# divyanshu-kumar/openh264-wasm

Hardware: AMD Instinct MI355X
Metric: 1080p30 frames/sec encode+decode per GPU (parity vs oracle; OpenH264 parity unpinned) (higher is better)
Workload: dtype u8

## Files before the change

openh264-wasm_amd/csrc/capi_enc.inc:

```
#include "../../include/h264mi.h"

namespace h264mi {
#define MAX_DECODERS 32
struct DecSlot { DecCtx *c; };
}

struct h264mi_instance {
    h264mi::EncCtx *encoder = nullptr;
    uint8_t *encoded_buffer = nullptr;
    int encoded_buffer_size = 0;
    uint8_t *rgba_dev = nullptr;
    size_t rgba_dev_size = 0;
    h264mi::DecSlot *decoder_pool[MAX_DECODERS] = {};
};

namespace h264mi {
static h264mi_instance g_instance;

static int enc_fetch(h264mi_instance *I, EncCtx *c, int s, uint8_t **out, int *out_size) {
    EncState st;
    if (hipMemcpyAsync(&st, c->d_st + s, sizeof(EncState), hipMemcpyDeviceToHost, c->stream) != hipSuccess) return 0;
    if (hipStreamSynchronize(c->stream) != hipSuccess) return 0;
    if (st.err || st.nal_bytes <= 0) return 0;
    if (I->encoded_buffer_size < st.nal_bytes) {
        free(I->encoded_buffer);
        I->encoded_buffer = (uint8_t *)malloc(st.nal_bytes);
        I->encoded_buffer_size = I->encoded_buffer ? st.nal_bytes : 0;
        if (!I->encoded_buffer) return 0;
    }
    const uint8_t *nal = c->h_desc[c->parity ^ 1][s].nal;
    if (hipMemcpy(I->encoded_buffer, nal, st.nal_bytes, hipMemcpyDeviceToHost) != hipSuccess) return 0;
    *out = I->encoded_buffer;
    *out_size = st.nal_bytes;
    return st.nal_bytes;
}
}

using namespace h264mi;

extern "C" {

int h264mi_i_init_encoder(h264mi_instance *I, int width, int height, int bitrate) {
    if (!I) return -1;
    if (I->encoder) { enc_free(I->encoder); I->encoder = nullptr; }
    I->encoder = enc_create(width, height, bitrate, 1, nullptr);
    return I->encoder ? 0 : -1;
}

void h264mi_i_force_key_frame(h264mi_instance *I) {
    if (I && I->encoder) {
        int one = 1;
        (void)hipMemcpyAsync(&I->encoder->d_st[0].force_idr, &one, sizeof(int), hipMemcpyHostToDevice, I->encoder->stream);
        (void)hipStreamSynchronize(I->encoder->stream);
        printf("Key frame forced.\n");
    }
}

void h264mi_i_encode_frame_yuv_i420(h264mi_instance *I, unsigned char *yuv, int width, int height, unsigned char **out_data,
                                    int *out_size) {
    *out_data = nullptr;
    *out_size = 0;
    EncCtx *c = I ? I->encoder : nullptr;
    if (!c || !yuv || width != c->w || height != c->h) return;
    if (hipMemcpyAsync(c->d_src, yuv, c->fbytes, hipMemcpyHostToDevice, c->stream) != hipSuccess) return;
    if (enc_frame(c, c->d_src) != 0) return;
    enc_fetch(I, c, 0, out_data, out_size);
}

void h264mi_i_encode_frame(h264mi_instance *I, unsigned char *rgba, int width, int height, unsigned char **out_data, int *out_size) {
    *out_data = nullptr;
    *out_size = 0;
    EncCtx *c = I ? I->encoder : nullptr;
    if (!c || !rgba || width != c->w || height != c->h) return;
    size_t n = (size_t)width * height * 4;
    if (I->rgba_dev_size < n) {
        (void)hipFree(I->rgba_dev);
        I->rgba_dev = nullptr; I->rgba_dev_size = 0;
        if (hipMalloc(&I->rgba_dev, n) != hipSuccess) return;
        I->rgba_dev_size = n;
    }
    if (hipMemcpyAsync(I->rgba_dev, rgba, n, hipMemcpyHostToDevice, c->stream) != hipSuccess) return;
    if (launch_rgba_to_i420(I->rgba_dev, width, height, 1, c->d_src, c->stream) != 0) return;
    if (enc_frame(c, c->d_src) != 0) return;
    enc_fetch(I, c, 0, out_data, out_size);
}

int init_encoder(int width, int height, int bitrate) { return h264mi_i_init_encoder(&g_instance, width, height, bitrate); }
void force_key_frame(void) { h264mi_i_force_key_frame(&g_instance); }
void encode_frame_yuv_i420(unsigned char *yuv, int width, int height, unsigned char **out_data, int *out_size) {
    h264mi_i_encode_frame_yuv_i420(&g_instance, yuv, width, height, out_data, out_size);
}
void encode_frame(unsigned char *rgba, int width, int height, unsigned char **out_data, int *out_size) {
    h264mi_i_encode_frame(&g_instance, rgba, width, height, out_data, out_size);
}

void free_buffer(void *ptr) {
    if (ptr != nullptr) free(ptr);
}

struct h264mi_encoder { EncCtx *c; };

h264mi_encoder *h264mi_enc_create(int width, int height, int bitrate, int nstreams, void *hip_stream) {
    EncCtx *c = enc_create(width, height, bitrate, nstreams, (hipStream_t)hip_stream);
    if (!c) return nullptr;
    return new h264mi_encoder{c};
}
void h264mi_enc_destroy(h264mi_encoder *e) {
    if (!e) return;
    (void)hipStreamSynchronize(e->c->stream);
    enc_free(e->c);
    delete e;
}
int h264mi_enc_force_idr(h264mi_encoder *e, int stream) {
    if (!e) return -1;
    int one = 1;
    for (int s = 0; s < e->c->S; s++)
        if (stream < 0 || s == stream)
            if (hipMemcpyAsync(&e->c->d_st[s].force_idr, &one, sizeof(int), hipMemcpyHostToDevice, e->c->stream) != hipSuccess) return -1;
    return hipStreamSynchronize(e->c->stream) == hipSuccess ? 0 : -1;
}
int h264mi_enc_set_frame_skip(h264mi_encoder *e, int enable) {
    if (!e) return -1;
    int v = enable != 0;
    for (int s = 0; s < e->c->S; s++)
        if (hipMemcpyAsync(&e->c->d_st[s].rc.skip_en, &v, sizeof(int), hipMemcpyHostToDevice, e->c->stream) != hipSuccess) return -1;
    return hipStreamSynchronize(e->c->stream) == hipSuccess ? 0 : -1;
}
int h264mi_enc_set_gom_exact(h264mi_encoder *e, int enable) {
    if (!e) return -1;
    if (enable && e->c->slices > 1) return -1;
    e->c->gom_exact = enable != 0;
    return 0;
}
int h264mi_enc_set_slices(h264mi_encoder *e, int n) {
    if (!e || !slices_valid(e->c->mbh, n) || (n > 1 && e->c->gom_exact)) return -1;
    e->c->slices = n;
    return 0;
}
int h264mi_enc_slices(h264mi_encoder *e) { return e ? e->c->slices : -1; }
int h264mi_slice_first_row(int mbh, int n, int k) {
    if (mbh < 1 || !slices_valid(mbh, n) || k < 0 || k > n) return -1;
    return slice_first_row(mbh, n, k);
}
int h264mi_enc_set_quality(h264mi_encoder *e, int enable) { return e ? enc_set_quality(e->c, enable != 0) : -1; }
int h264mi_enc_quality_enabled(h264mi_encoder *e) { return e ? (e->c->quality ? 1 : 0) : -1; }
int h264mi_enc_quality(h264mi_encoder *e, int stream, h264mi_quality *out) {
    if (!e || !out || !e->c->quality || stream < 0 || stream >= e->c->S) return -1;
    if (hipMemcpyAsync(out, e->c->d_qual + stream, sizeof(h264mi_quality), hipMemcpyDeviceToHost, e->c->stream) != hipSuccess) return -1;
    return hipStreamSynchronize(e->c->stream) == hipSuccess ? 0 : -1;
}
const h264mi_quality *h264mi_enc_quality_dev(h264mi_encoder *e) { return e && e->c->quality ? e->c->d_qual : nullptr; }
int h264mi_i420_quality_dev(h264mi_quality *d_out, const void *d_a, const void *d_b, int w, int h, int n, void *hip_stream) {
    if (!d_out || !d_a || !d_b || !quality_args_ok(w, h, n)) return -1;
    return launch_quality_i420(d_out, (const uint8_t *)d_a, (const uint8_t *)d_b, w, h, n, (hipStream_t)hip_stream);
}
double h264mi_psnr(uint64_t sse, uint64_t samples) {
    if (sse == 0) return 100.0;
    return 10.0 * log10(65025.0 * (double)samples / (double)sse);
}
int h264mi_enc_inject_error(h264mi_encoder *e, int stream, int code) {
    if (!e || stream < 0 || stream >= e->c->S || code <= 0) return -1;
    if (hipMemcpyAsync(&e->c->d_st[stream].inject_err, &code, sizeof(int), hipMemcpyHostToDevice, e->c->stream) != hipSuccess) return -1;
    return hipStreamSynchronize(e->c->stream) == hipSuccess ? 0 : -1;
}
int h264mi_enc_frames_skipped(h264mi_encoder *e, int stream) {
    if (!e || stream < 0 || stream >= e->c->S) return -1;
    EncState st;
    if (hipMemcpy(&st, e->c->d_st + stream, sizeof(EncState), hipMemcpyDeviceToHost) != hipSuccess) return -1;
    return st.skipped;
}
static int enc_blend_overlays(EncCtx *c) {
    if (c->ov.empty()) return 0;
    return launch_overlay_i420(c->d_src, c->w, c->h, c->ov_sprites, c->ov_w, c->ov_h, c->ov.data(), (int)c->ov.size(), c->stream);
}
int h264mi_enc_encode(h264mi_encoder *e, const void *d_frames) {
    if (!e || !d_frames) return -1;
    EncCtx *c = e->c;
    if (c->ov.empty()) return enc_frame(c, (const uint8_t *)d_frames);
    if (d_frames != (const void *)c->d_src) {
        const uintptr_t a = (uintptr_t)d_frames, b = (uintptr_t)c->d_src, nb = (uintptr_t)c->S * c->fbytes;
        if (a < b + nb && b < a + nb) return -1;
        if (hipMemcpyAsync(c->d_src, d_frames, nb, hipMemcpyDeviceToDevice, c->stream) != hipSuccess) return -1;
    }
    if (enc_blend_overlays(c) != 0) return -1;
    return enc_frame(c, c->d_src);
}
int h264mi_enc_set_overlays(h264mi_encoder *e, const void *d_sprites, int ow, int oh, int nsprites, const h264mi_overlay *ov, int nov) {
    if (!e) return -1;
    EncCtx *c = e->c;
    if (nov == 0) { c->ov.clear(); c->ov_sprites = nullptr; return 0; }
    if (!d_sprites || !overlay_args_ok(c->w, c->h, c->S, ow, oh, nsprites, ov, nov) ||
        overlay_ranges_overlap(c->d_src, c->w, c->h, c->S, d_sprites, ow, oh, nsprites))
        return -1;
    c->ov.assign(ov, ov + nov);
    c->ov_sprites = (const uint8_t *)d_sprites; c->ov_w = ow; c->ov_h = oh;
    return 0;
}
int h264mi_enc_overlays(h264mi_encoder *e) { return e ? (int)e->c->ov.size() : -1; }
int h264mi_rgba_to_i420a_dev(void *d_dst, const void *d_rgba, int w, int h, int n, void *hip_stream) {
    if (!d_dst || !d_rgba || ((uintptr_t)d_rgba & 3) || !rgba_to_i420a_args_ok(w, h, n)) return -1;
    return launch_rgba_to_i420a((const uint8_t *)d_rgba, w, h, n, (uint8_t *)d_dst, (hipStream_t)hip_stream);
}
int h264mi_i420_overlay_dev(void *d_canvas, int cw, int ch, int ncanvas, const void *d_sprites, int ow, int oh, int nsprites,
                            const h264mi_overlay *ov, int nov, void *hip_stream) {
    if (!d_canvas || !d_sprites || !overlay_args_ok(cw, ch, ncanvas, ow, oh, nsprites, ov, nov) ||
        overlay_ranges_overlap(d_canvas, cw, ch, ncanvas, d_sprites, ow, oh, nsprites))
        return -1;
    return launch_overlay_i420((uint8_t *)d_canvas, cw, ch, (const uint8_t *)d_sprites, ow, oh, ov, nov, (hipStream_t)hip_stream);
}
int h264mi_enc_encode_rgba(h264mi_encoder *e, const void *d_rgba_frames) {
    if (!e || !d_rgba_frames || ((uintptr_t)d_rgba_frames & 3)) return -1;
    EncCtx *c = e->c;
    if (launch_rgba_to_i420((const uint8_t *)d_rgba_frames, c->w, c->h, c->S, c->d_src, c->stream) != 0) return -1;
    if (enc_blend_overlays(c) != 0) return -1;
    return enc_frame(c, c->d_src);
}
int h264mi_i420_scale_dev(void *d_dst, int dw, int dh, const void *d_src, int sw, int sh, int n, void *hip_stream) {
    if (!d_dst || !d_src || !scale_args_ok(dw, dh, sw, sh, n) || scale_ranges_overlap(d_dst, dw, dh, d_src, sw, sh, n)) return -1;
    return launch_scale_i420((uint8_t *)d_dst, dw, dh, (const uint8_t *)d_src, sw, sh, n, (hipStream_t)hip_stream);
}
int h264mi_enc_encode_scaled(h264mi_encoder *e, const void *d_frames, int src_w, int src_h) {
    if (!e || !d_frames) return -1;
    EncCtx *c = e->c;
    if (!scale_args_ok(c->w, c->h, src_w, src_h, c->S) || scale_ranges_overlap(c->d_src, c->w, c->h, d_frames, src_w, src_h, c->S)) return -1;
    if (launch_scale_i420(c->d_src, c->w, c->h, (const uint8_t *)d_frames, src_w, src_h, c->S, c->stream) != 0) return -1;
    if (enc_blend_overlays(c) != 0) return -1;
    return enc_frame(c, c->d_src);
}
int h264mi_i420_compose_dev(void *d_canvas, int cw, int ch, int ncanvas, const void *d_src, int src_w, int src_h, int nsrc,
                            const h264mi_cell *cells, int ncells, void *hip_stream) {
    if (!d_canvas || !d_src || !compose_args_ok(cw, ch, ncanvas, src_w, src_h, nsrc, cells, ncells) ||
        compose_ranges_overlap(d_canvas, cw, ch, ncanvas, d_src, src_w, src_h, nsrc))
        return -1;
    return launch_compose_i420((uint8_t *)d_canvas, cw, ch, (const uint8_t *)d_src, src_w, src_h, cells, ncells, (hipStream_t)hip_stream);
}
int h264mi_i420_fill_dev(void *d_frames, int w, int h, int n, int y, int cb, int cr, void *hip_stream) {
    if (!d_frames || !fill_args_ok(w, h, n, y, cb, cr)) return -1;
    return launch_fill_i420((uint8_t *)d_frames, w, h, n, y, cb, cr, (hipStream_t)hip_stream);
}
int h264mi_mosaic_cells(h264mi_cell *out, int cap, int n, int src_w, int src_h, int cw, int ch) {
    return mosaic_cells(out, cap, n, src_w, src_h, cw, ch);
}
int h264mi_enc_encode_composed(h264mi_encoder *e, const void *d_src, int src_w, int src_h, int nsrc, const h264mi_cell *cells, int ncells,
                               int bg_y, int bg_cb, int bg_cr) {
    if (!e || !d_src) return -1;
    EncCtx *c = e->c;
    if (!compose_args_ok(c->w, c->h, c->S, src_w, src_h, nsrc, cells, ncells) ||
        compose_ranges_overlap(c->d_src, c->w, c->h, c->S, d_src, src_w, src_h, nsrc))
        return -1;
    if (bg_y > 255 || bg_cb > 255 || bg_cr > 255 || (bg_y >= 0 && !fill_args_ok(c->w, c->h, c->S, bg_y, bg_cb, bg_cr))) return -1;
    if (bg_y >= 0 && launch_fill_i420(c->d_src, c->w, c->h, c->S, bg_y, bg_cb, bg_cr, c->stream) != 0) return -1;
    if (launch_compose_i420(c->d_src, c->w, c->h, (const uint8_t *)d_src, src_w, src_h, cells, ncells, c->stream) != 0) return -1;
    if (enc_blend_overlays(c) != 0) return -1;
    return enc_frame(c, c->d_src);
}
int h264mi_i420_upscale_dev(void *d_dst, int dw, int dh, const void *d_src, int sw, int sh, int n, int filter, void *hip_stream) {
    if (!d_dst || !d_src || !upscale_args_ok(dw, dh, sw, sh, n, filter) || upscale_ranges_overlap(d_dst, dw, dh, d_src, sw, sh, n)) return -1;
    return launch_upscale_i420((uint8_t *)d_dst, dw, dh, (const uint8_t *)d_src, sw, sh, n, filter, (hipStream_t)hip_stream);
}
int h264mi_i420_compose_any_dev(void *d_canvas, int cw, int ch, int ncanvas, const void *d_src, int src_w, int src_h, int nsrc,
                                const h264mi_cell *cells, int ncells, int filter, void *hip_stream) {
    if (!d_canvas || !d_src || !compose_any_args_ok(cw, ch, ncanvas, src_w, src_h, nsrc, cells, ncells, filter) ||
        compose_ranges_overlap(d_canvas, cw, ch, ncanvas, d_src, src_w, src_h, nsrc))
        return -1;
    return launch_compose_any_i420((uint8_t *)d_canvas, cw, ch, (const uint8_t *)d_src, src_w, src_h, cells, ncells, filter,
                                   (hipStream_t)hip_stream);
}
int h264mi_speaker_cells(h264mi_cell *out, int cap, int n, int speaker, int src_w, int src_h, int cw, int ch) {
    return speaker_cells(out, cap, n, speaker, src_w, src_h, cw, ch);
}
int h264mi_enc_encode_composed_any(h264mi_encoder *e, const void *d_src, int src_w, int src_h, int nsrc, const h264mi_cell *cells, int ncells,
                                   int filter, int bg_y, int bg_cb, int bg_cr) {
    if (!e || !d_src) return -1;
    EncCtx *c = e->c;
    if (!compose_any_args_ok(c->w, c->h, c->S, src_w, src_h, nsrc, cells, ncells, filter) ||
        compose_ranges_overlap(c->d_src, c->w, c->h, c->S, d_src, src_w, src_h, nsrc))
        return -1;
    if (bg_y > 255 || bg_cb > 255 || bg_cr > 255 || (bg_y >= 0 && !fill_args_ok(c->w, c->h, c->S, bg_y, bg_cb, bg_cr))) return -1;
    if (bg_y >= 0 && launch_fill_i420(c->d_src, c->w, c->h, c->S, bg_y, bg_cb, bg_cr, c->stream) != 0) return -1;
    if (launch_compose_any_i420(c->d_src, c->w, c->h, (const uint8_t *)d_src, src_w, src_h, cells, ncells, filter, c->stream) != 0) return -1;
    if (enc_blend_overlays(c) != 0) return -1;
    return enc_frame(c, c->d_src);
}
const void *h264mi_enc_input_buffer(h264mi_encoder *e) { return e ? e->c->d_src : nullptr; }
size_t h264mi_enc_frame_bytes(h264mi_encoder *e) { return e ? e->c->fbytes : 0; }
size_t h264mi_enc_rgba_frame_bytes(h264mi_encoder *e) { return e ? (size_t)e->c->w * e->c->h * 4 : 0; }
int h264mi_enc_sync(h264mi_encoder *e) { return e && hipStreamSynchronize(e->c->stream) == hipSuccess ? 0 : -1; }
int h264mi_enc_nal_bytes(h264mi_encoder *e, int *out) {
    if (!e) return -1;
    std::vector<EncState> st(e->c->S);
    if (hipMemcpyAsync(st.data(), e->c->d_st, sizeof(EncState) * e->c->S, hipMemcpyDeviceToHost, e->c->stream) != hipSuccess) return -1;
    if (hipStreamSynchronize(e->c->stream) != hipSuccess) return -1;
    int err = 0;
    for (int s = 0; s < e->c->S; s++) { out[s] = st[s].nal_bytes; err |= st[s].err; }
    return err ? -2 : 0;
}
const void *h264mi_enc_nal_ptr(h264mi_encoder *e, int stream) {
    if (!e || stream < 0 || stream >= e->c->S) return nullptr;
    return e->c->h_desc[e->c->parity ^ 1][stream].nal;
}
const void *h264mi_enc_recon_ptr(h264mi_encoder *e, int stream) {
    if (!e || stream < 0 || stream >= e->c->S) return nullptr;
    return e->c->h_desc[e->c->parity ^ 1][stream].dbk[0];
}
int h264mi_enc_ref_planes(h264mi_encoder *e, int stream, void *host_out) {
    if (!e || stream < 0 || stream >= e->c->S) return -1;
    const EncDesc &d = e->c->h_desc[0][stream];
    const size_t lsz = (size_t)d.ps * (e->c->ch + 2 * H264MI_LPADY), csz = (size_t)d.psc * (e->c->ch / 2 + 2 * H264MI_CPADY);
    uint8_t *o = (uint8_t *)host_out;
    if (hipStreamSynchronize(e->c->stream) != hipSuccess) return -1;
    for (int k = 0; k < 4; k++)
        if (hipMemcpy(o + k * lsz, d.pl[k] - (size_t)H264MI_LPADY * d.ps - H264MI_LPADX, lsz, hipMemcpyDeviceToHost) != hipSuccess) return -1;
    for (int k = 0; k < 2; k++)
        if (hipMemcpy(o + 4 * lsz + k * csz, d.plc[k] - (size_t)H264MI_CPADY * d.psc - H264MI_CPADX, csz, hipMemcpyDeviceToHost) != hipSuccess) return -1;
    return 0;
}
int h264mi_enc_last_qp(h264mi_encoder *e, int stream) {
    if (!e || stream < 0 || stream >= e->c->S) return -1;
    EncState st;
    if (hipMemcpy(&st, e->c->d_st + stream, sizeof(EncState), hipMemcpyDeviceToHost) != hipSuccess) return -1;
    return st.cur_qp;
}
int h264mi_enc_rc_state(h264mi_encoder *e, int stream, int *out) {
    if (!e || !out || stream < 0 || stream >= e->c->S) return -1;
    EncState st;
    if (hipStreamSynchronize(e->c->stream) != hipSuccess) return -1;
    if (hipMemcpy(&st, e->c->d_st + stream, sizeof(EncState), hipMemcpyDeviceToHost) != hipSuccess) return -1;
    const RcState &r = st.rc;
    const int v[16] = {st.cur_skip, st.cur_qp, r.avg_qp, r.target, r.remaining, (int)r.fullness, r.continual_skip,
                       (int)r.frame_cmplx, r.min_frame_qp, r.max_frame_qp, r.bpf, r.pframe_num, r.idr_num, r.skip_flag,
                       r.remaining_weights, r.frame_coded_in_vgop};
    memcpy(out, v, sizeof(v));
    return 0;
}
int h264mi_enc_gom_state(h264mi_encoder *e, int stream, int *out, int cap) {
    if (!e || stream < 0 || stream >= e->c->S) return -1;
    const int G = e->c->gom_count;
    if (!out || !e->c->gom_exact) return G;
    if (hipStreamSynchronize(e->c->stream) != hipSuccess) return -1;
    std::vector<uint64_t> g(4 * (size_t)G);
    if (hipMemcpy(g.data(), e->c->h_desc[0][stream].gomst, 8 * g.size(), hipMemcpyDeviceToHost) != hipSuccess) return -1;
    for (int i = 0; i < 4 * G && i < cap; i++) out[i] = (int)(uint32_t)g[i];
    return G;
}
int h264mi_rc_qstep_to_qp(int qstep) {
    static const int32_t thr[52] = {H264MI_RC_QP_THR_LIST};
    if (qstep < 64) return 0;
    int q = 0;
    while (q < 52 && qstep >= thr[q]) q++;
    return q;
}
int h264mi_enc_mbinfo(h264mi_encoder *e, int stream, void *host_out) {
    if (!e || stream < 0 || stream >= e->c->S) return -1;
    return hipMemcpy(host_out, e->c->h_desc[0][stream].info, sizeof(MbInfo) * e->c->nmb, hipMemcpyDeviceToHost) == hipSuccess ? 0 : -1;
}
void *h264mi_enc_stream(h264mi_encoder *e) { return e ? (void *)e->c->stream : nullptr; }
const int *h264mi_enc_nal_size_dev(h264mi_encoder *e, int stream) {
    if (!e || stream < 0 || stream >= e->c->S) return nullptr;
    return &e->c->d_st[stream].nal_bytes;
}
int h264mi_enc_copy_nals(h264mi_encoder *e, void *d_dst, int slot_bytes, int *d_sizes) {
    if (!e || !d_dst || slot_bytes <= 0 || (slot_bytes & 3)) return -1;
    EncCtx *c = e->c;
    hipLaunchKernelGGL(enc_copy_nals_kernel, dim3(64, c->S), dim3(256), 0, c->stream,
                       PackNalLaunch{c->S, c->d_desc[c->parity ^ 1], (uint8_t *)d_dst, slot_bytes, (int32_t *)d_sizes});
    return hipGetLastError() == hipSuccess ? 0 : -1;
}
int h264mi_enc_profile(h264mi_encoder *e, uint64_t *out) {
    if (!e || !e->c->d_prof) return -1;
    return hipMemcpy(out, e->c->d_prof, 64 * sizeof(uint64_t), hipMemcpyDeviceToHost) == hipSuccess ? 0 : -1;
}
const uint32_t *h264mi_enc_rows_counter(h264mi_encoder *e) { return e ? e->c->d_ticket + 32 : nullptr; }
int h264mi_enc_timeline(h264mi_encoder *e, uint64_t *out, int n) {
    if (!e || !e->c->d_tl || n < 4 * e->c->S * e->c->mbh) return -1;
    return hipMemcpy(out, e->c->d_tl, 4 * (size_t)e->c->S * e->c->mbh * sizeof(uint64_t), hipMemcpyDeviceToHost) == hipSuccess ? 0 : -1;
}
int h264mi_enc_set_timing(h264mi_encoder *e, int enable) {
    if (!e) return -1;
    if (hipStreamSynchronize(e->c->stream) != hipSuccess) return -1;
    e->c->timing = enable != 0;
    e->c->ev_used = 0;
    return 0;
}
int h264mi_enc_kernel_time(h264mi_encoder *e, double *ms_total, int *launches) {
    if (!e) return -1;
    EncCtx *c = e->c;
    if (hipStreamSynchronize(c->stream) != hipSuccess) return -1;
    double t = 0;
    for (int i = 0; i + 1 < c->ev_used; i += 2) {
        float ms = 0;
        if (hipEventElapsedTime(&ms, c->ev[i], c->ev[i + 1]) != hipSuccess) return -1;
        t += ms;
    }
    *ms_total = t;
    *launches = c->ev_used / 2;
    return 0;
}

}
```

openh264-wasm_amd/csrc/enc_mb.inc:

```
namespace h264mi {

constexpr int ENC_THREADS = 256;
DEV int e_tid() { int t = threadIdx.x; asm volatile("" : "+v"(t)); return t; }
DEV int e_lane() { return e_tid() & 63; }
DEV int e_wave() { return threadIdx.x >> 6; }

constexpr int WIN_RING = 64, WINC_RING = 32;
constexpr int WIN_STRIDE = WIN_RING + 4, WINC_STRIDE = WINC_RING + 4;
DEV void win_put4(uint8_t *d, u32x4 v) { uint32_t *p = (uint32_t *)d; p[0] = v.x; p[1] = v.y; p[2] = v.z; p[3] = v.w; }
DEV void win_put2(uint8_t *d, u32x2 v) { uint32_t *p = (uint32_t *)d; p[0] = v.x; p[1] = v.y; }
constexpr int ENC_CROSS_THR = 1024;
struct EncLds {
    alignas(16) uint8_t win[4][64 * WIN_STRIDE];
    alignas(16) uint8_t winc[2][32 * WINC_STRIDE];
    alignas(16) uint8_t src[256];
    alignas(16) uint8_t srcc[2][64];
    alignas(16) uint8_t pred[256];
    alignas(16) uint8_t predc[2][64];
    alignas(16) uint8_t rec[256];
    alignas(16) uint8_t recc[2][64];
    uint8_t top[24];
    uint8_t topc[2][12];
    uint8_t left[16], leftc[2][8];
    uint8_t n4[16];
    alignas(16) int16_t lvl[24][16];
    alignas(16) int16_t ldc[16];
    alignas(16) int16_t cdc[2][4];
    int dcraw[24];
    int dcval[24];
    alignas(4) uint8_t nnz[24];
    alignas(4) int8_t i4[16];
    uint32_t gp[3][16];
    int cand[32];
    int pj[2][4];
    int refsk[H264MI_ENC_MAX_MBW];
    int abort_flag;
    int gom_qp;
    Xf xft[16];
    alignas(8) I4Tap i4t[9][16];
};

struct EncLaunch {
    int w, h, mbw, mbh, S;
    const EncDesc *desc;
    uint32_t *ticket;
    const uint8_t *src_base;
    size_t src_stride;
    uint64_t *prof;
    int src_vec;
    const DbkDesc *dbk;
    uint64_t *dprof;
    int dlag;
    int xq = 0;
    uint64_t *tl = nullptr;
    int prio = 0;
    int prof_row = -1;
    int gomr = 0;
    int sgrp = 0;
};

constexpr int HAD[4][4] = {{1, 1, 1, 1}, {1, 1, -1, -1}, {1, -1, -1, 1}, {1, -1, 1, -1}};
constexpr uint8_t INVZZ[16] = {0, 1, 5, 6, 2, 4, 7, 12, 3, 8, 11, 13, 9, 10, 14, 15};
constexpr int SUBDX[8] = {0, 0, -1, 1, -1, 1, -1, 1}, SUBDY[8] = {-1, 1, 0, 0, -1, -1, 1, 1};
constexpr uint32_t pack_sub(const int *v) { uint32_t r = 0; for (int k = 0; k < 8; k++) r |= (uint32_t)(v[k] + 1) << (2 * k); return r; }
constexpr uint32_t SUBDX_P = pack_sub(SUBDX), SUBDY_P = pack_sub(SUBDY);
DEV int sub_dx(int k) { return (int)((SUBDX_P >> (2 * k)) & 3) - 1; }
DEV int sub_dy(int k) { return (int)((SUBDY_P >> (2 * k)) & 3) - 1; }
struct QSel { int p1, dx1, dy1, p2, dx2, dy2; };
constexpr uint8_t QSEL_T[16][6] = {
    {0, 0, 0, 0, 0, 0}, {0, 0, 0, 1, 0, 0}, {1, 0, 0, 1, 0, 0}, {1, 0, 0, 0, 1, 0},
    {0, 0, 0, 2, 0, 0}, {1, 0, 0, 2, 0, 0}, {1, 0, 0, 3, 0, 0}, {1, 0, 0, 2, 1, 0},
    {2, 0, 0, 2, 0, 0}, {2, 0, 0, 3, 0, 0}, {3, 0, 0, 3, 0, 0}, {3, 0, 0, 2, 1, 0},
    {2, 0, 0, 0, 0, 1}, {2, 0, 0, 1, 0, 1}, {3, 0, 0, 1, 0, 1}, {2, 1, 0, 1, 0, 1}};
constexpr uint64_t pack_qsel(int half) {
    uint64_t r = 0;
    for (int i = 0; i < 8; i++) {
        const uint8_t *e = QSEL_T[8 * half + i];
        r |= (uint64_t)(e[0] | e[1] << 2 | e[2] << 3 | e[3] << 4 | e[4] << 6 | e[5] << 7) << (8 * i);
    }
    return r;
}
constexpr uint64_t QSEL_LO = pack_qsel(0), QSEL_HI = pack_qsel(1);
DEV QSel qsel(int idx) {
    const uint32_t e = (uint32_t)(((idx < 8 ? QSEL_LO : QSEL_HI) >> (8 * (idx & 7))) & 255);
    return QSel{(int)(e & 3), (int)((e >> 2) & 1), (int)((e >> 3) & 1), (int)((e >> 4) & 3), (int)((e >> 6) & 1), (int)(e >> 7)};
}

DEV int tap6(int a, int b, int c, int d, int e, int f) { return a - 5 * b + 20 * c + 20 * d - 5 * e + f; }

DEV int Wpl(const EncLds &S, int p, int Y0, int gx, int gy) { return S.win[p][(gy - Y0) * WIN_STRIDE + ((gx + 24) & (WIN_RING - 1))]; }
#define AVG(a, b) (((a) + (b) + 1) >> 1)
DEV int Wsample(const EncLds &S, int Y0, int gx, int gy, int fx, int fy) {
    const QSel q = qsel(fy * 4 + fx);
    return AVG(Wpl(S, q.p1, Y0, gx + q.dx1, gy + q.dy1), Wpl(S, q.p2, Y0, gx + q.dx2, gy + q.dy2));
}

DEV int chroma_mc_sample(const EncLds &S, int mbx, int mvx, int mvy, int pl, int x, int y) {
    const int fx = mvx & 7, fy = mvy & 7;
    const int X = mbx * 8 + (mvx >> 3), Y = (mvy >> 3) + 12;
    const uint8_t *W = S.winc[pl];
    const int r0 = (Y + y) * WINC_STRIDE, r1 = r0 + WINC_STRIDE, c0 = (X + x + 12) & (WINC_RING - 1), c1 = (X + x + 13) & (WINC_RING - 1);
    const int A = W[r0 + c0], B = W[r0 + c1], C = W[r1 + c0], E = W[r1 + c1];
    return ((8 - fx) * (8 - fy) * A + fx * (8 - fy) * B + (8 - fx) * fy * C + fx * fy * E + 32) >> 6;
}
DEV void chroma_mc(EncLds &S, int mbx, int mby, int mvx, int mvy) {
    for (int i = e_tid(); i < 128; i += ENC_THREADS) {
        const int pl = i >> 6, p = i & 63;
        S.predc[pl][p] = (uint8_t)chroma_mc_sample(S, mbx, mvx, mvy, pl, p & 7, p >> 3);
    }
}

}
```

openh264-wasm_amd/csrc/enc_mb_kernel.inc:

```
namespace h264mi {

DEV int code_residual_nodc(EncLds &S, const Xf &X, int qp, int intra, int do_luma, bool recon) {
    const int tid = e_tid(), pos = tid & 15, lane = tid & 63;
    const QuantQP q = make_qqp(qp), qc = make_qqp(c_CHROMA_QP[qp]);
    const int fl = qff(q, X.cls, intra), fc = qff(qc, X.cls, intra), fc0 = intra ? qc.fi0 : qc.fp0;
    const int lb = tid >> 4, lx = (lb & 3) * 4 + (pos & 3), ly = (lb >> 2) * 4 + (pos >> 2);
    if (do_luma) {
        const int pv = S.pred[ly * 16 + lx];
        const int t = xf_fwd(S.src[ly * 16 + lx] - pv, X);
        const int mf = X.cls == 0 ? q.mf0 : (X.cls == 1 ? q.mf1 : q.mf2);
        const int lv = quant1(t, mf, fl);
        S.lvl[lb][X.zz] = (int16_t)lv;
        const uint64_t m = __ballot(lv != 0);
        if (pos == 0) S.nnz[lb] = (int)popc((m >> (16 * (lb & 3))) & 0xffffu);
        if (recon) {
            const int v = X.cls == 0 ? q.v0 : (X.cls == 1 ? q.v1 : q.v2);
            const int r = (xf_inv((lv * v) << q.q6, X) + 32) >> 6;
            S.rec[ly * 16 + lx] = (uint8_t)clip1(pv + r);
        }
    }
    if (tid < 128) {
        const int cp = tid >> 6, cb = (tid >> 4) & 3, cx = (cb & 1) * 4 + (pos & 3), cy = (cb >> 1) * 4 + (pos >> 2);
        const int pv = S.predc[cp][cy * 8 + cx];
        const int t = xf_fwd(S.srcc[cp][cy * 8 + cx] - pv, X);
        const int mf = X.cls == 0 ? qc.mf0 : (X.cls == 1 ? qc.mf1 : qc.mf2);
        const int lvc = pos == 0 ? 0 : quant1(t, mf, fc);
        S.lvl[16 + 4 * cp + cb][X.zz] = (int16_t)lvc;
        const uint64_t mc = __ballot(lvc != 0);
        if (pos == 0) S.nnz[16 + 4 * cp + cb] = (int)popc((mc >> (16 * cb)) & 0xffffu);
        const int a = lane_read(t, 0), b = lane_read(t, 16), e = lane_read(t, 32), g = lane_read(t, 48);
        const int c0 = quant_dc(a + b + e + g, qc.mf0, fc0), c1 = quant_dc(a - b + e - g, qc.mf0, fc0);
        const int c2 = quant_dc(a + b - e - g, qc.mf0, fc0), c3 = quant_dc(a - b - e + g, qc.mf0, fc0);
        if (lane == 0) {
            S.cdc[cp][0] = (int16_t)c0; S.cdc[cp][1] = (int16_t)c1; S.cdc[cp][2] = (int16_t)c2; S.cdc[cp][3] = (int16_t)c3;
        }
        if (recon) {
            const int f = cb == 0 ? c0 + c1 + c2 + c3 : cb == 1 ? c0 - c1 + c2 - c3 : cb == 2 ? c0 + c1 - c2 - c3 : c0 - c1 - c2 + c3;
            const int v = X.cls == 0 ? qc.v0 : (X.cls == 1 ? qc.v1 : qc.v2);
            const int w = pos == 0 ? ((f * qc.v0) << qc.q6) >> 1 : (lvc * v) << qc.q6;
            const int r = (xf_inv(w, X) + 32) >> 6;
            S.recc[cp][cy * 8 + cx] = (uint8_t)clip1(pv + r);
        }
    }
    lds_barrier();
    const int probe = lane < 24 ? S.nnz[lane] : (lane < 32 ? S.cdc[(lane - 24) >> 2][(lane - 24) & 3] : 0);
    const uint32_t nzb = (uint32_t)__ballot(probe != 0);
    const int lum = ((nzb & 0x0033u) ? 1 : 0) | ((nzb & 0x00ccu) ? 2 : 0) | ((nzb & 0x3300u) ? 4 : 0) | ((nzb & 0xcc00u) ? 8 : 0);
    const int cbpc = (nzb & 0x00ff0000u) ? 2 : ((nzb & 0xff000000u) ? 1 : 0);
    return uni(lum | (cbpc << 4));
}
DEV int code_residual(EncLds &S, const Xf &X, int qp, int i16, int intra, int do_luma, bool recon = true) {
    const int tid = e_tid(), pos = tid & 15, lane = tid & 63;
    const QuantQP q = make_qqp(qp), qc = make_qqp(c_CHROMA_QP[qp]);
    const int fl = qff(q, X.cls, intra), fc = qff(qc, X.cls, intra), fc0 = intra ? qc.fi0 : qc.fp0;
    const int lb = tid >> 4, lx = (lb & 3) * 4 + (pos & 3), ly = (lb >> 2) * 4 + (pos >> 2);
    int lv = 0;
    if (do_luma) {
        const int d = S.src[ly * 16 + lx] - S.pred[ly * 16 + lx];
        const int t = xf_fwd(d, X);
        if (i16 && pos == 0) S.dcraw[lb] = t;
        const int mf = X.cls == 0 ? q.mf0 : (X.cls == 1 ? q.mf1 : q.mf2);
        lv = (i16 && pos == 0) ? 0 : quant1(t, mf, fl);
        S.lvl[lb][X.zz] = (int16_t)lv;
        const uint64_t m = __ballot(lv != 0);
        if (pos == 0) S.nnz[lb] = (int)popc((m >> (16 * (lb & 3))) & 0xffffu);
    }
    const bool isc = tid < 128;
    const int cp = (tid >> 6) & 1, cb = (tid >> 4) & 3, cx = (cb & 1) * 4 + (pos & 3), cy = (cb >> 1) * 4 + (pos >> 2);
    int lvc = 0;
    if (isc) {
        const int d = S.srcc[cp][cy * 8 + cx] - S.predc[cp][cy * 8 + cx];
        const int t = xf_fwd(d, X);
        if (pos == 0) S.dcraw[16 + 4 * cp + cb] = t;
        const int mf = X.cls == 0 ? qc.mf0 : (X.cls == 1 ? qc.mf1 : qc.mf2);
        lvc = pos == 0 ? 0 : quant1(t, mf, fc);
        S.lvl[16 + 4 * cp + cb][X.zz] = (int16_t)lvc;
    }
    const uint64_t mc = __ballot(lvc != 0);
    if (isc && pos == 0) S.nnz[16 + 4 * cp + cb] = (int)popc((mc >> (16 * cb)) & 0xffffu);
    lds_barrier();
    if (tid < 16 && i16) {
        const int F = (xf_had(S.dcraw[tid], X) + 1) >> 1;
        S.ldc[X.zz] = (int16_t)quant_dc(F, q.mf0, q.fi0);
    }
    if (tid >= 16 && tid < 24) {
        const int pl = (tid - 16) >> 2, k = (tid - 16) & 3;
        const int a = S.dcraw[16 + 4 * pl], b = S.dcraw[17 + 4 * pl], e = S.dcraw[18 + 4 * pl], g = S.dcraw[19 + 4 * pl];
        const int f = k == 0 ? a + b + e + g : k == 1 ? a - b + e - g : k == 2 ? a + b - e - g : a - b - e + g;
        S.cdc[pl][k] = (int16_t)quant_dc(f, qc.mf0, fc0);
    }
    lds_barrier();
    const int probe = lane < 24 ? S.nnz[lane] : (lane < 32 ? S.cdc[(lane - 24) >> 2][(lane - 24) & 3] : 0);
    const uint64_t nzm = __ballot(probe != 0);
    const uint32_t nzb = (uint32_t)nzm;
    int lum = ((nzb & 0x0033u) ? 1 : 0) | ((nzb & 0x00ccu) ? 2 : 0) | ((nzb & 0x3300u) ? 4 : 0) | ((nzb & 0xcc00u) ? 8 : 0);
    if (i16) lum = lum ? 15 : 0;
    const int cbpc = (nzb & 0x00ff0000u) ? 2 : ((nzb & 0xff000000u) ? 1 : 0);
    const int cbp = uni(lum | (cbpc << 4));
    if (!recon) return cbp;
    if (tid < 16 && i16) S.dcval[tid] = luma_dc_scale(xf_had(S.ldc[X.zz], X), q);
    if (tid >= 16 && tid < 24) {
        const int pl = (tid - 16) >> 2, k = (tid - 16) & 3;
        const int a = S.cdc[pl][0], b = S.cdc[pl][1], e = S.cdc[pl][2], g = S.cdc[pl][3];
        const int f = k == 0 ? a + b + e + g : k == 1 ? a - b + e - g : k == 2 ? a + b - e - g : a - b - e + g;
        S.dcval[16 + 4 * pl + k] = ((f * qc.v0) << qc.q6) >> 1;
    }
    lds_barrier();
    if (do_luma) {
        const int v = X.cls == 0 ? q.v0 : (X.cls == 1 ? q.v1 : q.v2);
        int w = (lv * v) << q.q6;
        if (i16 && pos == 0) w = S.dcval[lb];
        const int r = (xf_inv(w, X) + 32) >> 6;
        S.rec[ly * 16 + lx] = (uint8_t)clip1(S.pred[ly * 16 + lx] + r);
    }
    if (isc) {
        const int v = X.cls == 0 ? qc.v0 : (X.cls == 1 ? qc.v1 : qc.v2);
        int w = (lvc * v) << qc.q6;
        if (pos == 0) w = S.dcval[16 + 4 * cp + cb];
        const int r = (xf_inv(w, X) + 32) >> 6;
        S.recc[cp][cy * 8 + cx] = (uint8_t)clip1(S.predc[cp][cy * 8 + cx] + r);
    }
    lds_barrier();
    return cbp;
}

struct I16Ctx { int dc, a, b, c, has_top, has_left; };
template <class LDS> DEV I16Ctx i16_ctx(const LDS &S, int has_top, int has_left) {
    const int l = e_tid() & 15;
    const int st = S.top[1 + l], sl = S.left[l];
    const int hh = l < 8 ? (l + 1) * (S.top[9 + l] - S.top[7 - l]) : 0;
    const int vv = l < 8 ? (l + 1) * (S.left[8 + l] - (l < 7 ? S.left[6 - l] : S.top[0])) : 0;
    const int sumt = lane_read(group16_sum(st), 0), suml = lane_read(group16_sum(sl), 0);
    const int H = lane_read(group16_sum(hh), 0), V = lane_read(group16_sum(vv), 0);
    I16Ctx r;
    if (has_top && has_left) r.dc = (sumt + suml + 16) >> 5;
    else if (has_left) r.dc = (suml + 8) >> 4;
    else if (has_top) r.dc = (sumt + 8) >> 4;
    else r.dc = 128;
    r.a = uni(16 * (S.left[15] + S.top[16])); r.b = (5 * H + 32) >> 6; r.c = (5 * V + 32) >> 6;
    r.has_top = has_top; r.has_left = has_left;
    return r;
}
template <class LDS> DEV int i16_pred(const LDS &S, const I16Ctx &k, int mode, int x, int y) {
    int vh = mode == 0 ? S.top[1 + x] : S.left[y];
    int pln = clip1((k.a + k.b * (x - 7) + k.c * (y - 7) + 16) >> 5);
    return mode <= 1 ? vh : (mode == 2 ? k.dc : pln);
}
DEV bool i16_avail(const I16Ctx &k, int m) {
    return m == 2 || (m == 0 && k.has_top) || (m == 1 && k.has_left) || (m == 3 && k.has_top && k.has_left);
}
DEV void i16_fill_pred(EncLds &S, const I16Ctx &k, int mode) {
    for (int i = e_tid(); i < 256; i += ENC_THREADS) S.pred[i] = (uint8_t)i16_pred(S, k, mode, i & 15, i >> 4);
    lds_barrier();
}

DEV uint32_t md_i16_order(int flags) {
    switch (flags & 7) {
    case 1: case 5: return 0x20012u;
    case 2: case 6: return 0x20002u;
    case 3: return 0x30210u;
    case 7: return 0x43210u;
    default: return 0x10002u;
    }
}
DEV uint32_t md_chroma_order(int flags) {
    switch (flags & 7) {
    case 1: case 5: return 0x20010u;
    case 2: case 6: return 0x20020u;
    case 3: return 0x30012u;
    case 7: return 0x43012u;
    default: return 0x10000u;
    }
}
__constant__ uint64_t c_MD_I4_IDX4[16] = {
    0x7f7f7afa7f117a10ull, 0x7f7f7fff7f117f11ull, 0x7f7f7afa7f7f7afaull, 0x7f7f7fff7f7f7ffbull, 0x7f7f7afa7f117a14ull,
    0x7f7f7fff7f117f15ull, 0x7f7f7afa7f7f7afeull, 0x7f7f7fff7f7f7fffull, 0x7f7f7afa7f917a10ull, 0x7f7f7fff7f917f11ull,
    0x7f7f7afa7fff7afaull, 0x7f7f7fff7fff7ffbull, 0x7f7f7afa7f917a14ull, 0x7f7f7fff7f917f15ull, 0x7f7f7afa7fff7afeull,
    0x7f7f7fff7fff7fffull};
constexpr uint64_t MD_I4_CNT4 = 0x9431643172314231ull;
__constant__ uint32_t c_MD_I4_LIST4[16] = {0x2u, 0x812u, 0x2u, 0x8012u, 0x2u, 0x812u, 0x2u, 0x0u,
                                           0x2u, 0x812u, 0x7302u, 0x738012u, 0x2u, 0x812u, 0x7302u, 0x0u};
DEV int ue_bits(int v) { return 2 * (31 - __clz(v + 1)) + 1; }
DEV int md_first_min(uint32_t ord, const int *cost, int lam, int *best) {
    const int n = (int)(ord >> 16);
    int b = 0x7fffffff, bm = (int)(ord & 15u);
#pragma unroll
    for (int i = 0; i < 4; i++) {
        const int m = (int)((ord >> (4 * i)) & 15u);
        const int cm = m == 0 ? cost[0] : (m == 1 ? cost[1] : (m == 2 ? cost[2] : cost[3]));
        const int c = cm + lam * ue_bits(m);
        if (i < n && c < b) { b = c; bm = m; }
    }
    *best = b;
    return bm;
}
DEV int i4_choose(const int *c, int ai, int *cost) {
    const int cnt = (int)((MD_I4_CNT4 >> (4 * ai)) & 15u);
    int best, m;
    if (cnt == 7 || cnt == 9) {
        const bool hb = c[1] < c[2];
        best = hb ? c[1] : c[2]; m = hb ? 1 : 2;
        if (c[0] < best) { best = c[0]; m = 0; }
        if (c[0] < c[1]) {
            if (cnt == 9) {
                if (c[5] < best) { best = c[5]; m = 5; }
                if (best > c[7]) { best = c[7]; m = 7; }
                if (!(c[0] <= c[7] && c[0] <= c[5])) {
                    if (c[5] < c[7]) { if (c[4] < best) { best = c[4]; m = 4; } }
                    else if (c[3] < best) { best = c[3]; m = 3; }
                }
            } else {
                if (c[4] < best) { best = c[4]; m = 4; }
                if (c[5] < best) { best = c[5]; m = 5; }
            }
        } else {
            if (c[6] < best) { best = c[6]; m = 6; }
            if (best > c[8]) { best = c[8]; m = 8; }
            if (!(c[6] >= c[1] && c[8] >= c[1])) {
                if (c[8] > c[6]) { if (c[4] < best) { best = c[4]; m = 4; } }
                else if (cnt == 9 && c[3] < best) { best = c[3]; m = 3; }
            }
        }
    } else {
        best = 0x7fffffff; m = 2;
        const uint32_t list = c_MD_I4_LIST4[ai];
        for (int i = 0; i < cnt; i++) {
            const int mm = (int)((list >> (4 * i)) & 15u);
            if (c[mm] < best) { best = c[mm]; m = mm; }
        }
    }
    *cost = best;
    return m;
}
DEV void i16_sad_mode(EncLds &S, const I16Ctx &k, int m) {
    const int lane = e_lane(), blk = lane >> 2, row = lane & 3;
    const int y = (blk >> 2) * 4 + row, x0 = (blk & 3) * 4;
    if (!i16_avail(k, m)) return;
    const uint32_t sv = *(const uint32_t *)&S.src[y * 16 + x0];
    int v = 0;
#pragma unroll
    for (int j = 0; j < 4; j++) v += iabs((int)((sv >> (8 * j)) & 255) - i16_pred(S, k, m, x0 + j, y));
    const int sad = wave_sum(v);
    if (lane == 0) S.cand[20 + m] = sad;
}
DEV int i16_first_min(const EncLds &S, int lam, int flags, int *cost) {
    int c[4];
#pragma unroll
    for (int m = 0; m < 4; m++) c[m] = uni(S.cand[20 + m]);
    return md_first_min(md_i16_order(flags), c, lam, cost);
}
DEV int i16_decide_oh(EncLds &S, const I16Ctx &k, int lam, int flags, int *cost) {
    i16_sad_mode(S, k, uni(e_wave()));
    lds_barrier();
    return i16_first_min(S, lam, flags, cost);
}
DEV int vaa_intra_var(const EncLds &S) {
    const int l = e_lane() & 15, bx = l & 3, by = l >> 2;
    int t = 0;
#pragma unroll
    for (int y = 0; y < 4; y++) {
        const uint32_t w = *(const uint32_t *)&S.src[(4 * by + y) * 16 + 4 * bx];
        t += (int)(w & 255) + (int)((w >> 8) & 255) + (int)((w >> 16) & 255) + (int)(w >> 24);
    }
    const int a = t >> 4;
    const uint32_t sum = (uint32_t)lane_read(group16_sum(a), 0), sq = (uint32_t)lane_read(group16_sum(a * a), 0);
    return (int)(sq - ((sum * sum) >> 4));
}

struct CCtx { int a[2], b[2], c[2], has_top, has_left; };
template <class LDS> DEV CCtx chroma_ctx(const LDS &S, int has_top, int has_left) {
    CCtx r;
    for (int pl = 0; pl < 2; pl++) {
        int H = 0, V = 0;
        for (int i = 0; i < 4; i++) {
            H += (i + 1) * (S.topc[pl][1 + 4 + i] - S.topc[pl][1 + 2 - i]);
            V += (i + 1) * (S.leftc[pl][4 + i] - (2 - i >= 0 ? S.leftc[pl][2 - i] : S.topc[pl][0]));
        }
        r.a[pl] = uni(16 * (S.leftc[pl][7] + S.topc[pl][8])); r.b[pl] = uni((34 * H + 32) >> 6); r.c[pl] = uni((34 * V + 32) >> 6);
    }
    r.has_top = has_top; r.has_left = has_left;
    return r;
}
template <class LDS> DEV int chroma_dc_blk(const LDS &S, const CCtx &k, int pl, int bx, int by) {
    int st = 0, sl = 0;
    for (int i = 0; i < 4; i++) { st += S.topc[pl][1 + 4 * bx + i]; sl += S.leftc[pl][4 * by + i]; }
    int t = k.has_top, l = k.has_left;
    if (bx == by) return (t && l) ? (st + sl + 4) >> 3 : l ? (sl + 2) >> 2 : t ? (st + 2) >> 2 : 128;
    if (bx == 1) return t ? (st + 2) >> 2 : l ? (sl + 2) >> 2 : 128;
    return l ? (sl + 2) >> 2 : t ? (st + 2) >> 2 : 128;
}
template <class LDS> DEV int chroma_pred(const LDS &S, const CCtx &k, int mode, int pl, int x, int y, int dcv) {
    int hv = mode == 1 ? S.leftc[pl][y] : S.topc[pl][1 + x];
    const int ka = pl ? k.a[1] : k.a[0], kb = pl ? k.b[1] : k.b[0], kc = pl ? k.c[1] : k.c[0];
    int pln = clip1((ka + kb * (x - 3) + kc * (y - 3) + 16) >> 5);
    return mode == 0 ? dcv : (mode <= 2 ? hv : pln);
}
DEV bool chroma_avail(const CCtx &k, int m) {
    return m == 0 || (m == 1 && k.has_left) || (m == 2 && k.has_top) || (m == 3 && k.has_top && k.has_left);
}
__device__ __noinline__ int chroma_decide_fill(EncLds &S, int a0, int a1, int b0, int b1, int c0, int c1, int has_top, int has_left,
                                               int lam, int flags) {
    CCtx k;
    k.a[0] = uni(a0); k.a[1] = uni(a1); k.b[0] = uni(b0); k.b[1] = uni(b1); k.c[0] = uni(c0); k.c[1] = uni(c1);
    k.has_top = uni(has_top); k.has_left = uni(has_left);
    int lane = e_lane();
    int m = (lane >> 3) & 3, pl = (lane >> 2) & 1, blk = lane & 3, ox = (blk & 1) * 4, oy = (blk >> 1) * 4;
    int dcv = chroma_dc_blk(S, k, pl, blk & 1, blk >> 1);
    int d[16];
#pragma unroll
    for (int y = 0; y < 4; y++)
#pragma unroll
        for (int x = 0; x < 4; x++) d[4 * y + x] = S.srcc[pl][(oy + y) * 8 + ox + x] - chroma_pred(S, k, m, pl, ox + x, oy + y, dcv);
    int s = 0;
#pragma unroll
    for (int i = 0; i < 16; i++) s += iabs(d[i]);
    s = group8_sum(s);
    int c[4];
#pragma unroll
    for (int mm = 0; mm < 4; mm++) c[mm] = lane_read(s, mm * 8);
    int bc;
    int best = uni(md_first_min(md_chroma_order(uni(flags)), c, uni(lam), &bc));
    for (int i = e_tid(); i < 128; i += ENC_THREADS) {
        int p2 = i >> 6, p = i & 63, x = p & 7, y = p >> 3;
        int dv = chroma_dc_blk(S, k, p2, x >> 2, y >> 2);
        S.predc[p2][p] = (uint8_t)chroma_pred(S, k, best, p2, x, y, dv);
    }
    lds_barrier();
    return best;
}
DEV int chroma_decide_fill(EncLds &S, const CCtx &k, int lam, int flags) {
    return uni(chroma_decide_fill(S, k.a[0], k.a[1], k.b[0], k.b[1], k.c[0], k.c[1], k.has_top, k.has_left, lam, flags));
}

struct MvNb { int avail, ref, mx, my; };
DEV MvNb nb_from_payload(const uint32_t *p, int k, bool avail) {
    MvNb r;
    r.avail = avail;
    if (!avail) { r.ref = -1; r.mx = r.my = 0; return r; }
    r.ref = uni((int8_t)((p[8] >> (k < 2 ? 16 : 24)) & 255));
    r.mx = uni((int16_t)(p[12 + k] & 0xffff)); r.my = uni((int16_t)(p[12 + k] >> 16));
    return r;
}
DEV void mv_pred16(MvNb A, MvNb B, MvNb C, int out[2]) {
    if (!B.avail && !C.avail && A.avail) { B = A; C = A; }
    int n = (A.ref == 0) + (B.ref == 0) + (C.ref == 0);
    if (n == 1) {
        out[0] = A.ref == 0 ? A.mx : (B.ref == 0 ? B.mx : C.mx);
        out[1] = A.ref == 0 ? A.my : (B.ref == 0 ? B.my : C.my);
        return;
    }
    out[0] = median3(A.mx, B.mx, C.mx);
    out[1] = median3(A.my, B.my, C.my);
}
DEV bool me_start_cand(int n, int p0, int p1, int amx, int amy, int bmx, int bmy, int cmx, int cmy, bool okA, bool okB, bool okC,
                       int &cx, int &cy) {
    const int mx = n == 2 ? amx : (n == 3 ? bmx : cmx), my = n == 2 ? amy : (n == 3 ? bmy : cmy);
    const bool ok = n == 2 ? okA : (n == 3 ? okB : okC);
    const int vx = n == 0 ? p0 : (n == 1 ? 0 : mx), vy = n == 0 ? p1 : (n == 1 ? 0 : my);
    cx = clip3(-16, 16, (vx + 2) >> 2); cy = clip3(-16, 16, (vy + 2) >> 2);
    return n < 2 || ok;
}
DEV int mvbits(int mx, int my, const int mvp[2]) { return se_len(mx - mvp[0]) + se_len(my - mvp[1]); }

DEV uint32_t win4(const EncLds &S, int p, int wr, int gx) {
    const int sl = (gx + 24) & 63;
    const uint32_t *row = (const uint32_t *)&S.win[p][wr * WIN_STRIDE];
    return __builtin_amdgcn_alignbyte(row[((sl >> 2) + 1) & 15], row[sl >> 2], sl & 3);
}
DEV int sad16_row_group(const EncLds &S, int Y0, int X, int Y, int cx, int cy) {
    const int row = e_tid() & 15;
    const u32x4 sv = *(const u32x4 *)&S.src[row * 16];
    const int sl = (X + cx + 24) & 63, i0 = sl >> 2, sh = sl & 3;
    const uint32_t *rw = (const uint32_t *)&S.win[0][(Y + cy + row - Y0) * WIN_STRIDE];
    const uint32_t w0 = rw[i0], w1 = rw[(i0 + 1) & 15], w2 = rw[(i0 + 2) & 15], w3 = rw[(i0 + 3) & 15], w4 = rw[(i0 + 4) & 15];
    uint32_t acc = __builtin_amdgcn_sad_u8(sv.x, __builtin_amdgcn_alignbyte(w1, w0, sh), 0u);
    acc = __builtin_amdgcn_sad_u8(sv.y, __builtin_amdgcn_alignbyte(w2, w1, sh), acc);
    acc = __builtin_amdgcn_sad_u8(sv.z, __builtin_amdgcn_alignbyte(w3, w2, sh), acc);
    acc = __builtin_amdgcn_sad_u8(sv.w, __builtin_amdgcn_alignbyte(w4, w3, sh), acc);
    return group16_sum((int)acc);
}
template <int N> DEV void satd16_mv_n(const EncLds &S, int Y0, int X, int Y, const int *mvx, const int *mvy, int *out) {
    const int lane = e_tid() & 63, blk = lane >> 2, row = lane & 3;
    const int y = (blk >> 2) * 4 + row, x0 = (blk & 3) * 4;
    const uint32_t sv = *(const uint32_t *)&S.src[y * 16 + x0];
    const int s1 = (row & 1) ? -1 : 1, s2 = (row & 2) ? -1 : 1;
    int acc[N];
#pragma unroll
    for (int n = 0; n < N; n++) {
        const QSel q = qsel((mvy[n] & 3) * 4 + (mvx[n] & 3));
        const int gx = X + x0 + (mvx[n] >> 2), wr = Y + y + (mvy[n] >> 2) - Y0;
        const uint32_t pa = win4(S, q.p1, wr + q.dy1, gx + q.dx1), pb = win4(S, q.p2, wr + q.dy2, gx + q.dx2);
        const uint32_t pv = (pa | pb) - (((pa ^ pb) & 0xFEFEFEFEu) >> 1);
        const int d0 = (int)(sv & 255) - (int)(pv & 255), d1 = (int)((sv >> 8) & 255) - (int)((pv >> 8) & 255);
        const int d2 = (int)((sv >> 16) & 255) - (int)((pv >> 16) & 255), d3 = (int)(sv >> 24) - (int)(pv >> 24);
        const int a0 = d0 + d1, a1 = d0 - d1, a2 = d2 + d3, a3 = d2 - d3;
        int h0 = a0 + a2, h1 = a1 + a3, h2 = a0 - a2, h3 = a1 - a3;
        h0 = dpp<0xB1>(h0) + s1 * h0; h1 = dpp<0xB1>(h1) + s1 * h1; h2 = dpp<0xB1>(h2) + s1 * h2; h3 = dpp<0xB1>(h3) + s1 * h3;
        h0 = dpp<0x4E>(h0) + s2 * h0; h1 = dpp<0x4E>(h1) + s2 * h1; h2 = dpp<0x4E>(h2) + s2 * h2; h3 = dpp<0x4E>(h3) + s2 * h3;
        int v = iabs(h0) + iabs(h1) + iabs(h2) + iabs(h3);
        v += dpp<0xB1>(v);
        v += dpp<0x4E>(v);
        acc[n] = row == 0 ? (v + 1) >> 1 : 0;
    }
#pragma unroll
    for (int n = 0; n < N; n++) acc[n] = group16_sum(acc[n]);
#pragma unroll
    for (int n = 0; n < N; n++) out[n] = lane_read(acc[n], 0) + lane_read(acc[n], 16) + lane_read(acc[n], 32) + lane_read(acc[n], 48);
}
DEV int satd16_mv(const EncLds &S, int Y0, int X, int Y, int mvx, int mvy) {
    int r;
    satd16_mv_n<1>(S, Y0, X, Y, &mvx, &mvy, &r);
    return r;
}
#define PSKIP_MV_MIN (-29)
#define PSKIP_MV_MAX_LOW 12
#define PSKIP_MAX_LEVEL 1
#define PSKIP_LUMA_CTR_MAX 5
#define PSKIP_CHROMA_CTR_MAX 6
#define PSKIP_SINGLE_CTR 0x56Bu
DEV int single_ctr_lane(int lv, int zz) {
    const int m = group16_sum(lv != 0 ? 1 << zz : 0);
    const int lower = m & ((1 << zz) - 1);
    const int run = lower ? zz - 1 - (31 - __builtin_clz((unsigned)lower)) : zz;
    return lv != 0 ? (int)((PSKIP_SINGLE_CTR >> (2 * run)) & 3u) : 0;
}
DEV int zero_sad_bound(const QuantQP &q) {
    const int t0 = 65535 / q.mf0 - q.fp0, t1 = (65535 / q.mf1 - q.fp1) >> 2, t2 = (65535 / q.mf2 - q.fp2) >> 1;
    return min(t0, min(t1, t2));
}
DEV void pskip_luma(EncLds &S, const Xf &X, const QuantQP &q, int Y0, int MX, int MY, int mvx, int mvy, int lb, int &lsad, int &ctr,
                    bool &rej) {
    const int pos = e_lane() & 15, lx = (lb & 3) * 4 + (pos & 3), ly = (lb >> 2) * 4 + (pos >> 2);
    const int pv = Wsample(S, Y0, MX + lx + (mvx >> 2), MY + ly + (mvy >> 2), mvx & 3, mvy & 3);
    S.pred[ly * 16 + lx] = (uint8_t)pv;
    const int dl = S.src[ly * 16 + lx] - pv;
    const int bs = group16_sum(iabs(dl));
    lsad += lane_read(bs, 0) + lane_read(bs, 16) + lane_read(bs, 32) + lane_read(bs, 48);
    if (__ballot(bs > zero_sad_bound(q)) != 0) {
        const int lv = quant1(xf_fwd(dl, X), qmf(q, X.cls), qff(q, X.cls, 0));
        rej = rej || iabs(lv) > PSKIP_MAX_LEVEL;
#ifndef H264MI_DIAG_NO_CTR
        ctr += wave_sum(single_ctr_lane(lv, X.zz));
#endif
    }
}
DEV void pskip_chroma(EncLds &S, const Xf &X, const QuantQP &qc, int mbx, int mvx, int mvy, int cp, int &sad, bool &rej) {
    const int lane = e_lane(), pos = lane & 15, g = lane >> 4, cx = (g & 1) * 4 + (pos & 3), cy = (g >> 1) * 4 + (pos >> 2);
    const int pc = chroma_mc_sample(S, mbx, mvx, mvy, cp, cx, cy);
    S.predc[cp][cy * 8 + cx] = (uint8_t)pc;
    const int dc = S.srcc[cp][cy * 8 + cx] - pc;
    const int bs = group16_sum(iabs(dc));
    const int ps = lane_read(bs, 0) + lane_read(bs, 16) + lane_read(bs, 32) + lane_read(bs, 48);
    sad += ps;
    const int tdc = 65535 / (qc.mf0 >> 1) - 2 * qc.fp0;
    if (__ballot(bs > zero_sad_bound(qc)) != 0 || ps > tdc) {
        const int t = xf_fwd(dc, X);
        const int lvc = quant1(t, qmf(qc, X.cls), qff(qc, X.cls, 0));
        const int a = lane_read(t, 0), b = lane_read(t, 16), e = lane_read(t, 32), f = lane_read(t, 48);
        const bool dcnz = quant_dc(a + b + e + f, qc.mf0, qc.fp0) != 0 || quant_dc(a - b + e - f, qc.mf0, qc.fp0) != 0 ||
                          quant_dc(a + b - e - f, qc.mf0, qc.fp0) != 0 || quant_dc(a - b - e + f, qc.mf0, qc.fp0) != 0;
#ifndef H264MI_DIAG_NO_CTR
        const int cctr = wave_sum(single_ctr_lane(X.zz > 0 ? lvc : 0, X.zz > 0 ? X.zz - 1 : 0));
#else
        const int cctr = 0;
#endif
        rej = rej || iabs(lvc) > PSKIP_MAX_LEVEL || dcnz || cctr > PSKIP_CHROMA_CTR_MAX;
    }
}
DEV void pskip_publish(int *J, int lsad, int csad, int ctr, bool rej) {
    const int lane = e_lane();
    const bool r = __ballot(rej) != 0;
    if (lane == 0) {
        atomicAdd(&J[1], lsad + csad);
        atomicAdd(&J[3], lsad);
        if (ctr) atomicAdd(&J[2], ctr);
        if (r) atomicOr(&J[0], 1);
    }
}
DEV void pskip_judge_4w(EncLds &S, int *J, const Xf &X, int qp, int Y0, int MX, int MY, int mbx, int mvx, int mvy) {
    const int w = e_wave(), g = e_lane() >> 4;
    const QuantQP q = make_qqp(qp), qc = make_qqp(c_CHROMA_QP[qp]);
    int lsad = 0, csad = 0, ctr = 0;
    bool rej = false;
    pskip_luma(S, X, q, Y0, MX, MY, mvx, mvy, 4 * w + g, lsad, ctr, rej);
    if (w < 2) pskip_chroma(S, X, qc, mbx, mvx, mvy, w, csad, rej);
    pskip_publish(J, lsad, csad, ctr, rej);
}
DEV void pskip_judge_3w(EncLds &S, int *J, const Xf &X, int qp, int Y0, int MX, int MY, int mbx, int mvx, int mvy) {
    const int w = e_wave(), g = e_lane() >> 4;
    const QuantQP q = make_qqp(qp), qc = make_qqp(c_CHROMA_QP[qp]);
    int lsad = 0, csad = 0, ctr = 0;
    bool rej = false;
    pskip_luma(S, X, q, Y0, MX, MY, mvx, mvy, 4 * (w - 1) + g, lsad, ctr, rej);
    if (w == 1) pskip_luma(S, X, q, Y0, MX, MY, mvx, mvy, 12 + g, lsad, ctr, rej);
    else pskip_chroma(S, X, qc, mbx, mvx, mvy, w - 2, csad, rej);
    pskip_publish(J, lsad, csad, ctr, rej);
}
DEV int mb_pred_sad(EncLds &S, int *J, bool judged) {
    if (judged) return uni(J[1]);
    const int tid = e_tid();
    int v = iabs((int)S.src[tid] - (int)S.pred[tid]);
    if (tid < 128) v += iabs((int)S.srcc[tid >> 6][tid & 63] - (int)S.predc[tid >> 6][tid & 63]);
    v = wave_sum(v);
    if ((tid & 63) == 0) atomicAdd(&J[1], v);
    lds_barrier();
    return uni(J[1]);
}
DEV void fill_pred_mv(EncLds &S, int Y0, int X, int Y, int mvx, int mvy) {
    const int i = e_tid();
    S.pred[i] = (uint8_t)Wsample(S, Y0, X + (i & 15) + (mvx >> 2), Y + (i >> 4) + (mvy >> 2), mvx & 3, mvy & 3);
}

#define CAND(k) uni(S.cand[k])
DEV bool p_need1(int lane, bool has_next) {
    const int k = lane & 15;
    return (lane < 16 || (lane < 32 && has_next)) && (k == 8 || k >= 12);
}
#ifndef H264MI_ENC_REC_WAVE
#define H264MI_ENC_REC_WAVE 0
#endif
#ifndef H264MI_ENC_LATE_COMMIT
#define H264MI_ENC_LATE_COMMIT 0
#endif
#ifndef H264MI_ENC_ONEBAR
#define H264MI_ENC_ONEBAR 1
#endif
#ifndef H264MI_ENC_XF_LDS
#define H264MI_ENC_XF_LDS 1
#endif
#ifndef H264MI_ENC_ST2PF
#define H264MI_ENC_ST2PF 0
#endif
#ifndef H264MI_ENC_PH1
#define H264MI_ENC_PH1 1
#endif
#ifndef H264MI_ENC_LATE_PF
#define H264MI_ENC_LATE_PF 0
#endif
#ifndef H264MI_ENC_WPE
#define H264MI_ENC_WPE 4
#endif
template <bool LEAN>
__global__ __launch_bounds__(ENC_THREADS)
__attribute__((amdgpu_waves_per_eu(LEAN && H264MI_ENC_WPE > 0 ? H264MI_ENC_WPE : 1, LEAN && H264MI_ENC_WPE > 0 ? H264MI_ENC_WPE : 8)))
void enc_mb_kernel(EncLaunch a) {
    struct DbkCavlcLds { DbkLds d; CavlcTabs T; CavlcWaveLds w[2]; };
    static_assert(sizeof(DbkCavlcLds) <= sizeof(EncLds), "the deblocking workgroup fits the encoder's LDS");
    __shared__ union { EncLds e; DbkCavlcLds k; } SH;
    EncLds &S = SH.e;
    __shared__ int s_ticket;
    const int wv = threadIdx.x >> 6;
#define tid (LEAN ? e_tid() : (int)threadIdx.x)
#define lane (tid & 63)
    const int xq = a.xq, xqi = xq ? (int)(blockIdx.x & 7) : 0, Sq = xq ? a.S >> 3 : a.S;
    if (tid == 0) s_ticket = (int)atomicAdd(a.ticket + (xq ? 8 + xqi : 0), 1u);
    lds_barrier();
    const int t = uni(s_ticket), lagD = a.dlag;
    int tb, tsq;
    if (a.sgrp > 0 && a.sgrp < Sq) {
        const int per = 2 * a.mbh * a.sgrp, g = t / per, tt = t - g * per, gs = min(a.sgrp, Sq - g * a.sgrp);
        tb = tt / gs;
        tsq = g * a.sgrp + (tt - tb * gs);
    } else {
        tb = t / Sq;
        tsq = t - tb * Sq;
    }
    const int ts = xq ? tsq * 8 + xqi : tsq;
    const int tl_slot = xq ? xqi * 2 * Sq * a.mbh + t : t;
    if (a.tl && threadIdx.x == 0) a.tl[2 * tl_slot] = __builtin_amdgcn_s_memrealtime();
    auto tl_end = [&]() {
        if (a.tl && (threadIdx.x & 63) == 0)
            atomicMax((unsigned long long *)&a.tl[2 * tl_slot + 1], (unsigned long long)__builtin_amdgcn_s_memrealtime());
    };
    bool is_dbk;
    int trow;
    if (a.gomr > 0) {
        const int R = a.gomr, k = min(tb / (2 * R), (a.mbh - 1) / R), rows_k = min(R, a.mbh - k * R), ph = tb - 2 * R * k;
        is_dbk = ph >= rows_k;
        trow = k * R + (is_dbk ? ph - rows_k : ph);
    } else if (lagD <= 0 || lagD >= a.mbh) { is_dbk = tb >= a.mbh; trow = is_dbk ? tb - a.mbh : tb; }
    else if (tb < lagD) { is_dbk = false; trow = tb; }
    else {
        const int k = tb - lagD, m = 2 * (a.mbh - lagD);
        if (k < m) { is_dbk = !(k & 1); trow = is_dbk ? (k >> 1) : lagD + (k >> 1); }
        else { is_dbk = true; trow = (a.mbh - lagD) + (k - m); }
    }
    if (is_dbk) {
        const int dby = trow, dsi = ts;
        if (wv == 3 || dby >= a.mbh) return;
        if (uni(cst(a.desc)[dsi].st->cur_skip)) return;
        if (wv == 0) {
            CONSTANT const DbkDesc &DD = cst(a.dbk)[dsi];
            const DbkLaunch dl{a.mbw, a.mbh, a.S, a.dbk, nullptr, a.dprof};
            CONSTANT const EncDesc &DE = cst(a.desc)[dsi];
            const int nsl = uni(DE.st->cur_slices);
            deblock_row(SH.k.d, dl, DD, dby, DbkSrcGranules{gbl((const uint64_t *)DD.src_gran), a.mbw, dby, (uint32_t)uni((int)*DD.epoch),
                                                            gbl((const uint64_t *)DE.rowq), uni(DE.st->cur_qp),
                                                            slice_row_first(a.mbh, nsl, dby), dby > 0 && slice_row_first(a.mbh, nsl, dby - 1)});
        } else {
            CONSTANT const EncDesc &D = cst(a.desc)[dsi];
            cavlc_row(SH.k.T, SH.k.w[wv - 1], D, a.mbw, a.mbh, dby, wv - 1, 2, (uint32_t)uni((int)D.st->epoch), &D.st->err, a.gomr > 0);
        }
        tl_end();
        return;
    }
    const int mby = trow, sidx = ts;
    if (threadIdx.x == 0) __hip_atomic_fetch_add(a.ticket + 32, 1u, __ATOMIC_RELAXED, __HIP_MEMORY_SCOPE_AGENT);
    if (a.prio == 1) __builtin_amdgcn_s_setprio(1);
    else if (a.prio == 2) __builtin_amdgcn_s_setprio(2);
    else if (a.prio == 3) __builtin_amdgcn_s_setprio(3);
    else if (a.prio == 4 && (trow == 0 || trow == a.mbh - 1)) __builtin_amdgcn_s_setprio(3);
    else if (a.prio == 5 && (trow == 0 || trow == a.mbh - 1)) __builtin_amdgcn_s_setprio(2);
    CONSTANT const EncDesc &D = cst(a.desc)[sidx];
    EncState *st = D.st;
    const uint32_t epoch = (uint32_t)uni((int)st->epoch);
    const int mbw = a.mbw, cw = mbw * 16, ch = a.mbh * 16, w = a.w, h = a.h;
    if (uni(st->cur_skip)) {
        for (int pl = 0; pl < 3; pl++) {
            const int pw = pl ? cw / 2 : cw, rows = pl ? 8 : 16, n4 = pw / 4;
            GLOBAL const uint32_t *rs = (GLOBAL const uint32_t *)(gbl(D.ref[pl]) + (size_t)mby * rows * pw);
            GLOBAL uint32_t *rd = (GLOBAL uint32_t *)(gbl(D.dbk[pl]) + (size_t)mby * rows * pw);
            for (int i = tid; i < rows * n4; i += ENC_THREADS) rd[i] = rs[i];
        }
        GLOBAL const int32_t *ks = gbl(D.sksad_ref);
        GLOBAL int32_t *kd = gbl(D.sksad_cur);
        for (int i = tid; i < mbw; i += ENC_THREADS) kd[mby * mbw + i] = ks[mby * mbw + i];
        if (mby == 0 && tid == 0) kd[mbw * a.mbh] = ks[mbw * a.mbh];
        return;
    }
    const int idr = uni(st->cur_idr), slice_qp = uni(st->cur_qp);
    const int sl_row0 = slice_first_row(a.mbh, uni(st->cur_slices), slice_of_row(a.mbh, uni(st->cur_slices), mby));
    int32_t *abort_word = &st->err;
    int qp;
    if (a.gomr > 0 && !idr) {
        if (wv == 0) {
            const int g = gom_row_qp(D, st, mby, mbw, a.gomr, epoch, abort_word);
            if (lane == 0) S.gom_qp = g < 0 ? slice_qp : g;
        }
        lds_barrier();
        qp = uni(S.gom_qp);
    } else {
        qp = idr ? slice_qp : clip3(uni(st->rc.min_frame_qp), uni(st->rc.max_frame_qp), slice_qp + uni(gbl(D.rowqp)[mby]));
    }
    GLOBAL uint64_t *rowq = gbl(D.rowq);
    bool row_carried = false;
    const QuantQP q = make_qqp(qp);
    const int qpc = c_CHROMA_QP[qp];
    const QuantQP qc = make_qqp(qpc);
    const int lam = c_LAMBDA[qp];
#if H264MI_ENC_XF_LDS
    if (tid < 16) S.xft[tid] = xf_consts(tid);
#define XF (S.xft[e_tid() & 15])
#else
    const Xf XF = xf_consts(tid & 15);
#endif
    const int Y0 = mby * 16 - 24, Y = mby * 16;
    GLOBAL const uint8_t *srcY = gbl(a.src_base) + (size_t)sidx * a.src_stride, *srcU = srcY + (size_t)w * h, *srcV = srcU + (size_t)(w / 2) * (h / 2);
    GLOBAL uint64_t *const grow_prev = mby > sl_row0 ? gbl(D.gran) + (size_t)(mby - 1) * mbw * H264MI_GRANULES_PER_MB : nullptr;
#define above (grow_prev != nullptr)
    GLOBAL uint64_t *grow = gbl(D.gran) + (size_t)mby * mbw * H264MI_GRANULES_PER_MB;
    GLOBAL uint64_t *egr = gbl(D.egran);
    GLOBAL uint32_t *info32 = gbl((uint32_t *)D.info);
    GLOBAL MbCoef *coefg = gbl(D.coef);
    if (tid == 0) S.abort_flag = 0;
    int L_ref = -1, L_mvx = 0, L_mvy = 0;
    bool L_skip = false;
    int L_sksad = -1;
    bool i4_dirty = false;
    GLOBAL const int32_t *skref = gbl(D.sksad_ref) + (size_t)mby * mbw;
    const bool ref_p = !idr && uni(gbl(D.sksad_ref)[mbw * a.mbh]) != 0;
    if (ref_p)
        for (int i = tid; i < mbw; i += ENC_THREADS) S.refsk[i] = skref[i];
    if (mby == 0 && tid == 0) gbl(D.sksad_cur)[mbw * a.mbh] = idr ? 0 : 1;
    uint32_t L_i4 = 0;
    __shared__ uint64_t s_prof[40];
#if defined(H264MI_ENC_PROF_BUILD) || defined(H264MI_ENC_PROF_DETAIL)
    const bool prof = a.prof != nullptr && (a.prof_row < 0 || a.prof_row == mby);
#else
    constexpr bool prof = false;
#endif
    uint64_t t_prev = 0;
    if (prof) { if (tid < 40) s_prof[tid] = 0; t_prev = clock64(); }
    auto stamp = [&](int k, uint64_t t0) {
#ifdef H264MI_ENC_PROF_DETAIL
        if (prof && (threadIdx.x & 63) == 0) atomicAdd((unsigned long long *)&s_prof[k], (unsigned long long)(clock64() - t0));
#endif
    };
    auto lap = [&](int k) { if (prof) { uint64_t tt = clock64(); if (tid == 0) s_prof[k] += tt - t_prev; t_prev = tt; } };
#ifdef H264MI_ENC_FINE
    auto lapf = lap;
#else
    auto lapf = [](int) {};
#endif
    lds_barrier();

    const int ps = D.ps, psc = D.psc;
    GLOBAL const uint8_t *plw = gbl(D.pl[tid >> 6]) + (ptrdiff_t)(Y0 + (tid & 63)) * ps;
    GLOBAL const uint8_t *plcw = gbl(D.plc[(tid >> 5) & 1]) + (ptrdiff_t)(mby * 8 - 12 + (tid & 31)) * psc;
    const bool vsrc = a.src_vec != 0;
    u32x4 pfw = {0, 0, 0, 0}, pfa = {0, 0, 0, 0};
    auto issue_prefetch = [&](int nx) {
        if (!idr) {
            pfw = *(GLOBAL const u32x4 *)(plw + 16 * nx + 24);
            if (wv == 0) pfa.xy = *(GLOBAL const u32x2 *)(plcw + 8 * nx + 12);
        }
        if (vsrc && wv == 1) {
            if (lane < 16) pfa = *(GLOBAL const u32x4 *)(srcY + (size_t)min(Y + lane, h - 1) * w + 16 * nx);
            else if (lane < 32) {
                const int pl = (lane - 16) >> 3, r = (lane - 16) & 7;
                pfa.xy = *(GLOBAL const u32x2 *)((pl ? srcV : srcU) + (size_t)min(mby * 8 + r, h / 2 - 1) * (w / 2) + 8 * nx);
            }
        }
    };
    auto commit_prefetch = [&](int nx) {
        if (!idr) {
            win_put4(&S.win[tid >> 6][(tid & 63) * WIN_STRIDE + ((16 * nx + 48) & 63)], pfw);
            if (wv == 0) win_put2(&S.winc[lane >> 5][(lane & 31) * WINC_STRIDE + ((8 * nx + 24) & 31)], pfa.xy);
        }
        if (vsrc && wv == 1) {
            if (lane < 16) *(u32x4 *)&S.src[lane * 16] = pfa;
            else if (lane < 32) *(u32x2 *)&S.srcc[(lane - 16) >> 3][((lane - 16) & 7) * 8] = pfa.xy;
        }
    };
    auto load_src_bytes = [&](int mbx) {
        const int X = mbx * 16, i = tid;
        int x = min(X + (i & 15), w - 1), y = min(Y + (i >> 4), h - 1);
        S.src[i] = srcY[(size_t)y * w + x];
        if (tid < 128) {
            int pl = tid >> 6, p = tid & 63;
            x = min(mbx * 8 + (p & 7), w / 2 - 1); y = min(mby * 8 + (p >> 3), h / 2 - 1);
            S.srcc[pl][p] = (pl ? srcV : srcU)[(size_t)y * (w / 2) + x];
        }
    };
    if (!idr) {
#pragma unroll
        for (int k = 0; k < 4; k++)
            win_put4(&S.win[tid >> 6][(tid & 63) * WIN_STRIDE + 16 * k], *(GLOBAL const u32x4 *)(plw - 24 + 16 * k));
        if (wv == 0) {
#pragma unroll
            for (int k = 0; k < 4; k++)
                win_put2(&S.winc[lane >> 5][(lane & 31) * WINC_STRIDE + 8 * k], *(GLOBAL const u32x2 *)(plcw - 12 + 8 * k));
        }
    }
    load_src_bytes(0);
    if (tid < 16) { S.left[tid] = 0; S.leftc[tid >> 3][tid & 7] = 0; S.i4[tid] = 2; }
    if (tid < 8) S.pj[tid >> 2][tid & 3] = 0;
    static_assert(sizeof(I4Table) == 9 * 16 * 8, "I4Tap is 8 bytes");
    for (int i = tid; i < 9 * 16 * 2; i += ENC_THREADS) ((uint32_t *)S.i4t)[i] = ((const uint32_t *)&c_I4)[i];
    lds_barrier();

    int mbx_cur = 0;
    auto publish_decision = [&](int ty, int mx, int my, int sk) {
        if (wv == 1 && (lane == 8 || (lane >= 12 && lane < 16))) {
            const bool in = ty == MI_I4 || ty == MI_I16;
            const uint32_t v = lane == 8 ? (uint32_t)ty | ((uint32_t)qp << 8) | (in ? 0xffff0000u : 0u)
                                         : (lane == 13 ? (uint32_t)sk : (uint32_t)(uint16_t)mx | ((uint32_t)(uint16_t)my << 16));
            gran_store(grow + (size_t)mbx_cur * 16 + lane, epoch, v);
        }
    };
    uint64_t top_pf = 0;
    uint64_t st2_pf = 0;
    bool st2_stale = true;
    auto st2_need = [&](int nx) { return lane < 8 || lane == 9 || (nx > 0 && (lane == 19 || lane == 21 || lane == 23)); };
    auto st2_load = [&](int nx) -> uint64_t {
        return st2_need(nx) ? __hip_atomic_load(grow_prev + (size_t)(lane < 16 ? nx : nx - 1) * 16 + (lane & 15), __ATOMIC_RELAXED,
                                                __HIP_MEMORY_SCOPE_AGENT)
                            : 0;
    };
    int pend127 = -1;
    for (int mbx = 0; mbx < mbw; mbx++) {
        const int X = mbx * 16;
        mbx_cur = mbx;
        auto commit_here = [&]() {
            if (H264MI_ENC_LATE_COMMIT && mbx > 0) {
                commit_prefetch(mbx);
                stamp(20 + wv, t_prev);
            }
        };
        if (wv != 0 || !above) commit_here();
        if (above) {
            if (wv == 0) {
                bool ok = true;
                if (idr) {
                    uint32_t v;
                    if (mbx == 0) {
                        ok = gran_wait(grow_prev, 16, epoch, &v, abort_word);
                        if (ok && lane < 16) S.gp[0][lane] = v;
                    }
                    if (ok && mbx + 1 < mbw) {
                        ok = gran_wait(grow_prev + (size_t)(mbx + 1) * 16, 16, epoch, &v, abort_word);
                        if (ok && lane < 16) S.gp[(mbx + 1) % 3][lane] = v;
                    }
                } else {
                    const bool need = p_need1(lane, mbx + 1 < mbw);
#if H264MI_ENC_ST2PF
                    if (mbx == 0) st2_pf = st2_load(0);
#endif
                    if (mbx == 0) top_pf = need ? __hip_atomic_load(grow_prev + lane, __ATOMIC_RELAXED, __HIP_MEMORY_SCOPE_AGENT) : 0;
                    ok = gran_poll(grow_prev + (size_t)mbx * 16 + lane, need, epoch, top_pf, abort_word);
                    if (ok && need) S.gp[(mbx + (lane >> 4)) % 3][lane & 15] = (uint32_t)top_pf;
#if H264MI_ENC_ST2PF
                    {
                        const bool need2 = st2_need(mbx), fresh = (uint32_t)(st2_pf >> 32) == epoch;
                        if (ok && need2 && fresh) S.gp[(lane < 16 ? mbx : mbx - 1) % 3][lane & 15] = (uint32_t)st2_pf;
                        st2_stale = __ballot(need2 && !fresh) != 0;
                    }
#endif
                }
                if (!ok && lane == 0) S.abort_flag = 1;
                commit_here();
            }
            lds_barrier();
            if (S.abort_flag) return;
        }
        lap(mbx == 0 ? 0 : 1);
        const int ref_sk = ref_p ? uni(S.refsk[mbx]) : -1;
        if (mbx + 1 < mbw && (idr || !H264MI_ENC_LATE_PF)) issue_prefetch(mbx + 1);
        if (!vsrc && mbx > 0) load_src_bytes(mbx);
        const bool has_top = above, has_left = mbx > 0, has_tr = above && mbx + 1 < mbw, has_tl = has_top && has_left;
        const int nbf = (int)has_left | ((int)has_top << 1) | ((int)has_tl << 2) | ((int)has_tr << 3);
        const uint32_t *PB = S.gp[mbx % 3], *PC = S.gp[(mbx + 1) % 3], *PD = S.gp[(mbx + 2) % 3];
        auto fill_top = [&](bool all_waves, bool tr) {
            const int i = all_waves ? lane : tid;
            const bool luma = i < 21, chroma = i >= 32 && i < 50;
            const int pl = (i - 32) / 9, k = (i - 32) - 9 * pl;
            const int g = luma ? (i == 0 ? 2 * 16 + 3 : (i <= 16 ? (i - 1) >> 2 : 16 + ((i - 17) >> 2)))
                               : (chroma ? (k == 0 ? 2 * 16 + 5 + 2 * pl : 4 + 2 * pl + ((k - 1) >> 2)) : 0);
            const uint32_t w = S.gp[(mbx + (g >> 4)) % 3][g & 15];
            const int sh = luma ? (i == 0 ? 24 : 8 * ((i - 1) & 3)) : (k == 0 ? 24 : 8 * ((k - 1) & 3));
            const bool av = luma ? (i == 0 ? has_tl : (i <= 16 ? has_top : (has_tr && tr))) : (k == 0 ? has_tl : has_top);
            const uint8_t v = av ? (uint8_t)(w >> sh) : (uint8_t)0;
            if (luma) S.top[i] = v;
            if (chroma) S.topc[pl][k] = v;
        };
        auto poll_above = [&](bool tr) -> bool {
            if (!above || (tr && !has_tr)) return true;
            if (wv == 0 && (tr || !H264MI_ENC_ST2PF || st2_stale)) {
#ifndef H264MI_DIAG_NO_G9
                const bool need = tr ? lane < 4 : (lane < 8 || lane == 9 || (mbx > 0 && (lane == 19 || lane == 21 || lane == 23)));
#else
                const bool need = tr ? lane < 4 : (lane < 8 || (mbx > 0 && (lane == 19 || lane == 21 || lane == 23)));
#endif
                const int nb = tr ? mbx + 1 : (lane < 16 ? mbx : mbx - 1);
                GLOBAL uint64_t *g = grow_prev + (size_t)nb * 16 + (lane & 15);
                uint64_t x = need ? __hip_atomic_load(g, __ATOMIC_RELAXED, __HIP_MEMORY_SCOPE_AGENT) : 0;
                const bool ok = gran_poll(g, need, epoch, x, abort_word);
                if (ok && need) S.gp[nb % 3][lane & 15] = (uint32_t)x;
                if (!ok && lane == 0) S.abort_flag = 1;
            }
            lds_barrier();
            return !S.abort_flag;
        };
        if (idr) fill_top(false, true);
        if (idr || i4_dirty) {
            if (tid < 16) S.i4[tid] = 2;
        }
        if (idr || !vsrc || i4_dirty) lds_barrier();
        i4_dirty = false;

        int type = MI_I16, cbp = 0, i16mode = 0, cmode = 0, mvx = 0, mvy = 0, mvdx = 0, mvdy = 0;
        int cur_sk = -1;
        int *J = S.pj[mbx & 1];
        lap(2);
        bool do_intra = idr;
        I16Ctx k16;
        int m16 = 0, c16 = 0x7fffffff;
        if (idr) {
            k16 = i16_ctx(S, has_top, has_left);
            m16 = i16_decide_oh(S, k16, lam, nbf, &c16);
        } else {
#ifdef H264MI_ISA_MARK
            asm volatile(";;MARK_PSTART" ::: "memory");
#endif
            MvNb A, B, C;
            A.avail = has_left;
            if (has_left) { A.ref = L_ref; A.mx = L_mvx; A.my = L_mvy; } else { A.ref = -1; A.mx = A.my = 0; }
            B = nb_from_payload(PB, 0, has_top);
            C = has_tr ? nb_from_payload(PC, 0, true) : nb_from_payload(PD, 3, has_tl);
            int mvp[2], skmv[2] = {0, 0};
            mv_pred16(A, B, C, mvp);
            if (has_left && has_top && !(A.ref == 0 && A.mx == 0 && A.my == 0) && !(B.ref == 0 && B.mx == 0 && B.my == 0)) {
                skmv[0] = mvp[0]; skmv[1] = mvp[1];
            }
            const bool skA = has_left && L_skip, skB = has_top && (uni((int)PB[8]) & 255) == MI_PSKIP;
            const bool skC = has_tr && (uni((int)PC[8]) & 255) == MI_PSKIP, skD = has_tl && (uni((int)PD[8]) & 255) == MI_PSKIP;
            const bool ref_skip = ref_p && ref_sk >= 0;
            const int sx = (skmv[0] >> 2) + 16 * mbx, sy = (skmv[1] >> 2) + 16 * mby;
#ifndef H264MI_DIAG_ALWAYS_TRY
            const bool try_skip = (skA || skB || skC || skD || ref_skip) && sx >= PSKIP_MV_MIN && sx <= ((16 * mbw) | PSKIP_MV_MAX_LOW) &&
                                  sy >= PSKIP_MV_MIN && sy <= ((16 * a.mbh) | PSKIP_MV_MAX_LOW);
#else
            const bool try_skip = true;
#endif
            auto pskip_take = [&]() -> bool {
                const int sA = skA ? L_sksad : 0, sB = skB ? uni((int)PB[13]) : 0;
                const bool skCC = has_tr ? skC : skD;
                const int sC = skCC ? uni((int)(has_tr ? PC[13] : PD[13])) : 0;
                const int f = (int)skA | ((int)skB << 1) | ((int)skCC << 2);
                const int pred = (!has_top && !has_tl && has_left) ? sA : (f == 1 ? sA : (f == 2 ? sB : (f == 4 ? sC : median3(sA, sB, sC))));
                const int tsad = uni(J[1]);
                const bool res_ok = uni(J[0]) == 0 && uni(J[2]) <= PSKIP_LUMA_CTR_MAX;
                return tsad == 0 || tsad < pred || (ref_skip && tsad < ref_sk) || res_ok;
            };
            const bool pred_skip = has_left ? L_skip : skB;
            const bool beside = try_skip && !pred_skip;
            bool skip_taken = false;
            if (H264MI_ENC_LATE_PF == 2 && mbx + 1 < mbw) issue_prefetch(mbx + 1);
#ifdef H264MI_ISA_MARK
            asm volatile(";;MARK_JUDGE" ::: "memory");
#endif
            if (try_skip && pred_skip) {
                pskip_judge_4w(S, J, XF, qp, Y0, X, Y, mbx, skmv[0], skmv[1]);
                lds_barrier();
                skip_taken = pskip_take();
            }
            const bool me_ran = !skip_taken;
            if (!skip_taken) {
                if (!poll_above(false)) return;
#if H264MI_ENC_PH1 == 0
                fill_top(false, false);
                lds_barrier();
                k16 = i16_ctx(S, has_top, has_left);
#elif H264MI_ENC_PH1 == 1
                fill_top(true, false);
                k16 = i16_ctx(S, has_top, has_left);
#endif
#ifdef H264MI_ENC_PROF_DETAIL
                const uint64_t t_ph = prof ? clock64() : 0;
#else
                const uint64_t t_ph = 0;
#endif
                if (wv != 0) {
#if H264MI_ENC_PH1 == 0
                    if (beside) pskip_judge_3w(S, J, XF, qp, Y0, X, Y, mbx, skmv[0], skmv[1]);
                    i16_sad_mode(S, k16, uni(wv - 1));
                    if (wv == (beside ? 3 : 1)) i16_sad_mode(S, k16, 3);
#else
                    if (beside) {
                        pskip_judge_3w(S, J, XF, qp, Y0, X, Y, mbx, skmv[0], skmv[1]);
                        stamp(24 + wv, t_ph);
#if H264MI_ENC_PH1 == 2
                        fill_top(true, false);
                        k16 = i16_ctx(S, has_top, has_left);
#endif
                        if (wv == 1) i16_sad_mode(S, k16, 1);
                        stamp(28 + wv, t_ph);
                        if (wv == 1) i16_sad_mode(S, k16, 0);
                        else if (wv == 3) i16_sad_mode(S, k16, 3);
                        stamp(32 + wv, t_ph);
                    } else {
#if H264MI_ENC_PH1 == 2
                        fill_top(true, false);
                        k16 = i16_ctx(S, has_top, has_left);
#endif
                        i16_sad_mode(S, k16, uni(wv - 1));
                        if (wv == 1) i16_sad_mode(S, k16, 3);
                    }
#endif
                } else {
                    const int grp = (tid >> 4) & 3;
                    int bx, by, bc;
                    {
                        const bool okA = A.avail & (A.ref == 0), okB = B.avail & (B.ref == 0), okC = C.avail & (C.ref == 0);
                        const int amx = A.mx, amy = A.my, bmx = B.mx, bmy = B.my, cmx = C.mx, cmy = C.my, p0 = mvp[0], p1 = mvp[1];
                        auto cand_xy = [&](int n, int &cx, int &cy) -> bool {
                            return me_start_cand(n, p0, p1, amx, amy, bmx, bmy, cmx, cmy, okA, okB, okC, cx, cy);
                        };
                        int cx, cy;
                        bool av = cand_xy(grp, cx, cy);
                        int cost = sad16_row_group(S, Y0, X, Y, cx, cy) + lam * mvbits(4 * cx, 4 * cy, mvp);
                        int k = wave_min(av ? (cost << 3) | grp : 0x7fffffff);
                        if (uni((int)okC)) {
                            av = cand_xy(4, cx, cy) && grp == 0;
                            cost = sad16_row_group(S, Y0, X, Y, cx, cy) + lam * mvbits(4 * cx, 4 * cy, mvp);
                            k = min(k, wave_min(av ? (cost << 3) | 4 : 0x7fffffff));
                        }
                        bc = k >> 3;
                        cand_xy(k & 7, bx, by);
                    }
                    if (beside) stamp(24, t_ph);
                    lapf(12);
                    for (int it = 0; it < 32; it++) {
                        const int cx = bx + (grp == 1 ? -1 : (grp == 2 ? 1 : 0)), cy = by + (grp == 0 ? -1 : (grp == 3 ? 1 : 0));
                        const int sad = sad16_row_group(S, Y0, X, Y, cx, cy);
                        const bool ok = cx >= -16 && cx <= 16 && cy >= -16 && cy <= 16;
                        const int k = wave_min(ok ? ((sad + lam * mvbits(4 * cx, 4 * cy, mvp)) << 2) | grp : 0x7fffffff);
                        if (k == 0x7fffffff || (k >> 2) >= bc) break;
                        bc = k >> 2;
                        bx += (k & 3) == 1 ? -1 : ((k & 3) == 2 ? 1 : 0);
                        by += (k & 3) == 0 ? -1 : ((k & 3) == 3 ? 1 : 0);
                    }
                    if (lane == 0) { S.cand[17] = bx; S.cand[18] = by; S.cand[19] = bc; }
#if H264MI_ENC_PH1 == 2
                    fill_top(true, false);
                    k16 = i16_ctx(S, has_top, has_left);
#endif
#if H264MI_ENC_PH1 != 0
                    if (beside) {
                        stamp(28, t_ph);
                        i16_sad_mode(S, k16, 2);
                        stamp(32, t_ph);
                    }
#endif
                }
#ifndef H264MI_ENC_FINE
                if (prof && lane == 0) atomicAdd((unsigned long long *)&s_prof[11 + wv], (unsigned long long)(clock64() - t_prev));
#endif
                lds_barrier();
                if (beside) skip_taken = pskip_take();
            }
            if (H264MI_ENC_LATE_PF == 1 && mbx + 1 < mbw) issue_prefetch(mbx + 1);
            lap(3);
#ifndef H264MI_DIAG_NO_SKIP_INTRA
            if (skip_taken && !(skA && skB && skC)) {
#else
            if (false) {
#endif
                if (!me_ran) {
                    if (!poll_above(false)) return;
                    fill_top(true, false);
                    k16 = i16_ctx(S, has_top, has_left);
                    i16_sad_mode(S, k16, uni(wv));
                    lds_barrier();
                }
                m16 = i16_first_min(S, lam, nbf, &c16);
                do_intra = c16 < uni(J[3]);
            }
            if (skip_taken && !do_intra) {
                type = MI_PSKIP; mvx = skmv[0]; mvy = skmv[1]; cbp = 0;
                cur_sk = uni(J[1]);
                publish_decision(type, mvx, mvy, cur_sk);
            } else if (!skip_taken) {
                int bx = uni(S.cand[17]), by = uni(S.cand[18]), bcf = uni(S.cand[19]);
                if (uni(S.cand[19]) > ENC_CROSS_THR) {
                    const int bc = uni(S.cand[19]);
                    int kl = 0x7fffffff;
#pragma unroll 1
                    for (int pass = 0; pass < 4; pass++) {
                        const int j = pass * 16 + ((tid >> 4) & 15), hz = j < 32, i = hz ? j : j - 32;
                        const int t = i - 16 + (i - 16 >= (hz ? bx : by) ? 1 : 0);
                        const int cx = hz ? t : bx, cy = hz ? by : t, k = hz ? t + 16 : t + 49;
                        const int sad = sad16_row_group(S, Y0, X, Y, cx, cy);
                        kl = min(kl, ((sad + lam * mvbits(4 * cx, 4 * cy, mvp)) << 7) | k);
                    }
                    const int kmin = wave_min(kl);
                    if (lane == 0) S.cand[24 + wv] = kmin;
                    lds_barrier();
                    const int km = min(min(uni(S.cand[24]), uni(S.cand[25])), min(uni(S.cand[26]), uni(S.cand[27])));
                    if ((km >> 7) < bc) {
                        const int k = km & 127;
                        if (k < 33) bx = k - 16; else by = k - 49;
                        bcf = km >> 7;
                    }
                }
                lap(4);
                m16 = i16_first_min(S, lam, nbf, &c16);
                do_intra = c16 < bcf;
              if (!do_intra) {
                const int wv4 = uni(tid >> 6);
                {
                    int mx[3], my[3], cv[3];
#pragma unroll
                    for (int n = 0; n < 3; n++) {
                        const int k = wv4 + 4 * n - 1;
                        mx[n] = 4 * bx + (k < 0 ? 0 : 2 * sub_dx(k & 7)); my[n] = 4 * by + (k < 0 ? 0 : 2 * sub_dy(k & 7));
                    }
                    if (wv4 == 0) {
                        satd16_mv_n<3>(S, Y0, X, Y, mx, my, cv);
                        if (lane == 0) { S.cand[0] = cv[0]; S.cand[4] = cv[1]; S.cand[8] = cv[2]; }
                    } else {
                        satd16_mv_n<2>(S, Y0, X, Y, mx, my, cv);
                        if (lane == 0) { S.cand[wv4] = cv[0]; S.cand[wv4 + 4] = cv[1]; }
                    }
                }
                lds_barrier();
                lapf(13);
                int bdx, bdy, sc;
                {
                    const int k = lane - 1, ddx = lane == 0 ? 0 : 2 * sub_dx(k & 7), ddy = lane == 0 ? 0 : 2 * sub_dy(k & 7);
                    const int key = lane < 9 ? ((S.cand[lane] + lam * mvbits(4 * bx + ddx, 4 * by + ddy, mvp)) << 4) | lane : 0x7fffffff;
                    const int m = wave_min(key), o = m & 15;
                    sc = m >> 4;
                    bdx = o == 0 ? 0 : 2 * sub_dx(o - 1); bdy = o == 0 ? 0 : 2 * sub_dy(o - 1);
                }
                {
                    int mx[2], my[2], cv[2];
#pragma unroll
                    for (int n = 0; n < 2; n++) { mx[n] = 4 * bx + bdx + sub_dx(wv4 + 4 * n); my[n] = 4 * by + bdy + sub_dy(wv4 + 4 * n); }
                    satd16_mv_n<2>(S, Y0, X, Y, mx, my, cv);
                    if (lane == 0) { S.cand[9 + wv4] = cv[0]; S.cand[13 + wv4] = cv[1]; }
                }
                lds_barrier();
                lapf(14);
                {
                    const int ddx = bdx + sub_dx(lane & 7), ddy = bdy + sub_dy(lane & 7);
                    const int key = lane < 8 ? ((S.cand[9 + lane] + lam * mvbits(4 * bx + ddx, 4 * by + ddy, mvp)) << 4) | (lane + 1)
                                             : (lane == 8 ? sc << 4 : 0x7fffffff);
                    const int m = wave_min(key), o = m & 15;
                    sc = m >> 4;
                    if (o > 0) { bdx += sub_dx(o - 1); bdy += sub_dy(o - 1); }
                }
                lap(5);
                {
                    type = MI_P16x16;
                    mvx = 4 * bx + bdx; mvy = 4 * by + bdy;
                    const bool at_skmv = mvx == skmv[0] && mvy == skmv[1];
                    if (!at_skmv) publish_decision(type, mvx, mvy, -1);
                    mvdx = mvx - mvp[0]; mvdy = mvy - mvp[1];
                    fill_pred_mv(S, Y0, X, Y, mvx, mvy);
                    chroma_mc(S, mbx, mby, mvx, mvy);
                    lapf(15);
                    cbp = code_residual_nodc(S, XF, qp, 0, 1, true);
                    if (at_skmv) {
                        if (cbp == 0) { type = MI_PSKIP; cur_sk = mb_pred_sad(S, J, try_skip); }
                        publish_decision(type, mvx, mvy, cur_sk);
                    }
                }
                lap(7);
              }
            }
        }
        if (do_intra) {
            if (!idr) publish_decision(MI_I16, 0, 0, -1);
            int cost4 = 0;
            bool won = vaa_intra_var(S) > 149;
            if (!idr && won) {
                if (!poll_above(true)) return;
                fill_top(false, true);
                lds_barrier();
            }
            for (int blk = 0; won && blk < 16; blk++) {
                const int ras = (blk & 8) | ((blk & 2) << 1) | ((blk & 4) >> 1) | (blk & 1), bx = ras & 3, by = ras >> 2, ox = bx * 4, oy = by * 4;
                const bool bt = by > 0 || has_top, bl = bx > 0 || has_left;
                bool btr;
                if (by == 0) btr = bx < 3 ? has_top : has_tr;
                else btr = (bx < 3) && ras != 5 && ras != 13;
                if (tid < 13) {
                    int v = 0;
                    if (lane == 0) {
                        if (bt && bl) v = (bx > 0 && by > 0) ? S.rec[(oy - 1) * 16 + ox - 1] : (by > 0 ? S.left[oy - 1] : S.top[ox]);
                    } else if (lane <= 8) {
                        int i = lane - 1;
                        if (bt) {
                            int ii = (i >= 4 && !btr) ? 3 : i;
                            v = by > 0 ? S.rec[(oy - 1) * 16 + ox + ii] : S.top[1 + ox + ii];
                        }
                    } else {
                        int i = lane - 9;
                        if (bl) v = bx > 0 ? S.rec[(oy + i) * 16 + ox - 1] : S.left[oy + i];
                    }
                    S.n4[lane] = (uint8_t)v;
                }
                lds_barrier();
                const int ma = uni(bx > 0 ? S.i4[ras - 1] : (has_left ? (int)(int8_t)(L_i4 >> (8 * by)) : -1));
                const int mb = uni(by > 0 ? S.i4[ras - 4] : (has_top ? (int)(int8_t)((PB[9] >> (8 * bx)) & 255) : -1));
                const int pm = (ma < 0 || mb < 0) ? 2 : min(ma, mb);
                const int s4t = S.n4[1] + S.n4[2] + S.n4[3] + S.n4[4], s4l = S.n4[9] + S.n4[10] + S.n4[11] + S.n4[12];
                const int dcv = (bt && bl) ? (s4t + s4l + 4) >> 3 : bl ? (s4l + 2) >> 2 : bt ? (s4t + 2) >> 2 : 128;
                int cm[9];
                {
                    const int p = lane & 15, g = lane >> 4;
                    const int sv = S.src[(oy + (p >> 2)) * 16 + ox + (p & 3)];
#pragma unroll
                    for (int k = 0; k < 3; k++) {
                        const int m = 4 * k + g;
                        const int pv = m == 2 ? dcv : i4_tap_eval(S.i4t[m < 9 ? m : 8][p], S.n4);
                        const int sad = group16_sum(iabs(sv - pv));
#pragma unroll
                        for (int gg = 0; gg < 4; gg++)
                            if (4 * k + gg < 9) cm[4 * k + gg] = lane_read(sad, 16 * gg) + ((4 * k + gg) == pm ? lam : lam << 2);
                    }
                }
                int bcost;
                const int best = i4_choose(cm, (int)((c_MD_I4_IDX4[nbf] >> (4 * blk)) & 15u), &bcost);
                cost4 += bcost;
                if (cost4 >= c16) { won = false; break; }
                if (wv == 0) {
                    const int p = lane & 15, o = (oy + (p >> 2)) * 16 + ox + (p & 3);
                    const int pv = best == 2 ? dcv : i4_tap_eval(S.i4t[best][p], S.n4);
                    const int t = xf_fwd(S.src[o] - pv, XF);
                    const int lv = quant1(t, qmf(q, XF.cls), qff(q, XF.cls, 1));
                    const int n = (int)popc(__ballot(lv != 0) & 0xffffu);
                    const int r = (xf_inv((lv * (XF.cls == 0 ? q.v0 : (XF.cls == 1 ? q.v1 : q.v2))) << q.q6, XF) + 32) >> 6;
                    if (lane < 16) {
                        S.rec[o] = (uint8_t)clip1(pv + r);
                        S.lvl[ras][XF.zz] = (int16_t)lv;
                    }
                    if (lane == 0) { S.nnz[ras] = n; S.i4[ras] = (int8_t)best; }
                }
                lds_barrier();
            }
            lap(8);
            won = won && cost4 + 24 * lam < c16;
            const CCtx kc = chroma_ctx(S, has_top, has_left);
            if (won) {
                type = MI_I4;
                cmode = chroma_decide_fill(S, kc, lam, nbf);
                cbp = code_residual_nodc(S, XF, qp, 1, 0, true);
            } else {
                type = MI_I16; i16mode = m16;
                if (tid < 16) S.i4[tid] = 2;
                i16_fill_pred(S, k16, m16);
                cmode = chroma_decide_fill(S, kc, lam, nbf);
                cbp = code_residual(S, XF, qp, 1, 1, 1);
            }
            if (!idr) i4_dirty = type == MI_I4;
            lap(9);
        }
        if (!H264MI_ENC_LATE_COMMIT && mbx + 1 < mbw) {
            commit_prefetch(mbx + 1);
            stamp(20 + wv, t_prev);
        }
        if (!idr && wv == 0 && above && mbx + 1 < mbw) {
            const bool need = p_need1(lane, mbx + 2 < mbw);
#if H264MI_ENC_ST2PF
            st2_pf = st2_load(mbx + 1);
#endif
            top_pf = need ? __hip_atomic_load(grow_prev + (size_t)(mbx + 1) * 16 + lane, __ATOMIC_RELAXED, __HIP_MEMORY_SCOPE_AGENT) : 0;
        }
        const int mbi = mby * mbw + mbx;
        const bool intra = type == MI_I4 || type == MI_I16, skip = type == MI_PSKIP;
        const uint32_t mvw = (uint32_t)(uint16_t)mvx | ((uint32_t)(uint16_t)mvy << 16), refw = intra ? 0xffffffffu : 0u;
        constexpr int O_I4 = offsetof(EncLds, i4) / 4, O_NZ = offsetof(EncLds, nnz) / 4;
        const int O_REC = skip ? (int)(offsetof(EncLds, pred) / 4) : (int)(offsetof(EncLds, rec) / 4);
        const int O_RECC = skip ? (int)(offsetof(EncLds, predc) / 4) : (int)(offsetof(EncLds, recc) / 4);
        const uint8_t *LB = (const uint8_t *)&S;
        auto ldsw = [&](int dw) -> uint32_t { return ((const uint32_t *)&S)[dw]; };
        const bool carries = type == MI_I16 || (!skip && cbp != 0);
        const uint32_t qflag = (row_carried || carries) ? 0u : 0x80u;
        if (wv == H264MI_ENC_REC_WAVE && lane == 0 && carries && !row_carried && mby + 1 < a.mbh) gran_store(rowq + mby + 1, epoch, (uint32_t)qp);
        row_carried = row_carried || carries;
        if (wv == H264MI_ENC_REC_WAVE && lane < 32) {
            const uint32_t ld = ldsw(lane >= 2 && lane < 6 ? O_I4 + lane - 2 : (lane >= 7 && lane < 13 ? O_NZ + lane - 7 : O_I4));
            uint32_t v = (lane == 14 || lane == 31) ? 0u : mvw;
            if (lane == 0) v = (uint32_t)type | (((uint32_t)qp | qflag) << 8) | ((uint32_t)cbp << 16) | ((uint32_t)i16mode << 24);
            if (lane == 1) v = (uint32_t)cmode | (((uint32_t)qpc | qflag) << 8);
            if (lane >= 2 && lane < 6) v = ld;
            if (lane == 6) v = refw;
            if (lane >= 7 && lane < 13) v = skip ? 0u : ld;
            if (lane == 13) v = (uint32_t)(uint16_t)mvdx | ((uint32_t)(uint16_t)mvdy << 16);
            if (lane < 31) info32[(size_t)mbi * 32 + lane] = v;
            if (lane < 31) gran_store(egr + (size_t)mbi * 128 + 96 + lane, epoch, v);
        }
        if (wv == H264MI_ENC_REC_WAVE) stamp(36, t_prev);
        if (wv == 1 && lane < 16 && (idr || !(lane == 8 || lane >= 12))) {
            const uint32_t ld = ldsw(lane < 4 ? O_REC + 60 + lane
                                              : (lane < 8 ? O_RECC + 16 * ((lane - 4) >> 1) + 14 + (lane & 1)
                                                          : (lane == 9 ? O_I4 + 3 : (lane == 10 ? O_NZ + 3 : O_NZ + 4))));
            const uint32_t ld5 = ldsw(O_NZ + 5);
            uint32_t v = mvw;
            if (lane < 8 || lane == 9) v = ld;
            if (lane == 8) v = (uint32_t)type | ((uint32_t)qp << 8) | (refw & 0xffff0000u);
            if (lane == 10) v = skip ? 0u : ld;
            if (lane == 11) v = skip ? 0u : ((ld >> 16) | (ld5 & 0xffff0000u));
            gran_store(grow + (size_t)mbx * 16 + lane, epoch, v);
        }
        if (wv == 1) stamp(37, t_prev);
        if (wv == 2) {
            if (pend127 >= 0) {
                asm volatile("s_waitcnt vmcnt(0)" ::: "memory");
                if (lane == 0) gran_store(egr + (size_t)pend127 * 128 + 127, epoch, 0u);
            }
            stamp(38, t_prev);
            const int blk = lane >> 1, half = lane & 1;
            const int16_t *src = nullptr;
            int dst8 = 0;
            if (!skip && lane < 52) {
                if (blk < 16 && S.nnz[blk]) { src = S.lvl[blk]; dst8 = 4 * blk; }
                else if (blk >= 16 && blk < 24 && S.nnz[blk] && (cbp >> 4) == 2) { src = S.lvl[blk]; dst8 = 64 + 4 * (blk - 16); }
                else if (blk == 24 && type == MI_I16) { src = S.ldc; dst8 = 96; }
                else if (blk == 25 && (cbp >> 4) && half == 0) { src = &S.cdc[0][0]; dst8 = 100; }
            }
            if (src) {
                const u32x4 v = *(const u32x4 *)(src + 8 * half);
                const auto rsrc = __builtin_amdgcn_make_buffer_rsrc((void *)(uint64_t)(coefg + mbi), (short)0, 0x7fffffff, 0x00020000);
                __builtin_amdgcn_raw_buffer_store_b128(v, rsrc, (dst8 + 2 * half) * 8, 0, 16);
            }
            pend127 = mbi;
        }
        if (wv == 3 && lane < 48) {
            const uint32_t *pw = (const uint32_t *)LB + (lane < 32 ? O_REC + 2 * lane : O_RECC + 16 * ((lane - 32) >> 3) + ((lane - 32) & 7) * 2);
            gran_store2(egr + (size_t)mbi * 128, lane < 32 ? 2 * lane : 64 + 2 * (lane - 32), epoch, pw[0], pw[1]);
        }
        if (wv == 3) stamp(39, t_prev);
        L_ref = intra ? -1 : 0; L_mvx = mvx; L_mvy = mvy; L_skip = skip; L_sksad = cur_sk;
        if (!idr && wv == 3 && lane == 63) gbl(D.sksad_cur)[mbi] = cur_sk;
        L_i4 = (uint32_t)uni((int)((uint32_t)(uint8_t)S.i4[3] | ((uint32_t)(uint8_t)S.i4[7] << 8) | ((uint32_t)(uint8_t)S.i4[11] << 16) |
                                   ((uint32_t)(uint8_t)S.i4[15] << 24)));
        stamp(16 + wv, t_prev);
#if H264MI_ENC_ONEBAR
        if (tid < 16) S.left[lane] = LB[4 * O_REC + lane * 16 + 15];
        else if (tid < 32) S.leftc[(lane - 16) >> 3][lane & 7] = LB[4 * O_RECC + 64 * ((lane - 16) >> 3) + (lane & 7) * 8 + 7];
        else if (tid >= 32 && tid < 36) S.pj[(mbx + 1) & 1][tid - 32] = 0;
        lds_barrier();
#else
        lds_barrier();
        if (tid < 16) S.left[lane] = LB[4 * O_REC + lane * 16 + 15];
        else if (tid < 32) S.leftc[(lane - 16) >> 3][lane & 7] = LB[4 * O_RECC + 64 * ((lane - 16) >> 3) + (lane & 7) * 8 + 7];
        else if (tid >= 32 && tid < 36) S.pj[(mbx + 1) & 1][tid - 32] = 0;
        lds_barrier();
#endif
        lap(10);
    }
    if (wv == 2 && pend127 >= 0) {
        asm volatile("s_waitcnt vmcnt(0)" ::: "memory");
        if (lane == 0) gran_store(egr + (size_t)pend127 * 128 + 127, epoch, 0u);
    }
    if (!row_carried && mby + 1 < a.mbh && wv == 0) {
        int eq;
        if (row_entry_qp(rowq, mby, !above, slice_qp, epoch, abort_word, &eq) && lane == 0) gran_store(rowq + mby + 1, epoch, (uint32_t)eq);
    }
    if (prof && tid < 40) atomicAdd((unsigned long long *)&a.prof[tid < 16 ? tid : tid + 16], (unsigned long long)s_prof[tid]);
    tl_end();
#undef tid
#undef lane
#undef above
#if H264MI_ENC_XF_LDS
#undef XF
#endif
}

}
```

openh264-wasm_amd/csrc/enc_planes.inc:

```
namespace h264mi {

struct PlanesLaunch { int S, cw, ch; const PlanesDesc *pd; int ystrips; };

constexpr int PT_H = 16, PT_Q = 256;
static_assert((2 * H264MI_LPADY) % PT_H == 0, "planes strips tile the padded height");
DEV uint32_t planes_row_bytes(const uint8_t *row, int x, int cw) {
    const uint32_t v = *(const uint32_t *)(row + clip3(0, cw - 4, x));
    return x < 0 ? (v & 255u) * 0x01010101u : (x >= cw ? (v >> 24) * 0x01010101u : v);
}
DEV void ref_planes_chroma(const PlanesLaunch &a, const PlanesDesc &D, int i);
DEV void ref_planes_block(const PlanesLaunch &a, int bx, int by, int bz, int gx) {
    const PlanesDesc &D = a.pd[bz];
    if (D.active && *D.active == 0) return;
    if (by >= a.ystrips) {
        ref_planes_chroma(a, D, ((by - a.ystrips) * gx + bx) * PT_Q + (int)threadIdx.x);
        return;
    }
    const int cw = a.cw, ch = a.ch;
    const int pw = cw + 2 * H264MI_LPADX;
    const int q = bx * PT_Q + (int)threadIdx.x;
    if (q * 4 >= pw) return;
    const int x0 = q * 4 - H264MI_LPADX;
    const int ya = by * PT_H - H264MI_LPADY;
    const uint8_t *ref = D.src[D.parity ? (*D.parity & 1) : 0][0];
    uint32_t Mw[6], Bw[6][2], qL, qM, qR;
    auto issue = [&](int i) {
        const uint8_t *row = ref + (size_t)clip3(0, ch - 1, ya - 2 + i) * cw;
        qL = planes_row_bytes(row, x0 - 4, cw);
        qM = planes_row_bytes(row, x0, cw);
        qR = planes_row_bytes(row, x0 + 4, cw);
    };
    auto absorb = [&](int slot) {
        const uint32_t lo = __builtin_amdgcn_alignbyte(qM, qL, 2), hi = __builtin_amdgcn_alignbyte(qR, qM, 2);
        int sm[9];
        sm[0] = lo & 255; sm[1] = (lo >> 8) & 255; sm[2] = (lo >> 16) & 255; sm[3] = lo >> 24;
        sm[4] = hi & 255; sm[5] = (hi >> 8) & 255; sm[6] = (hi >> 16) & 255; sm[7] = hi >> 24; sm[8] = (qR >> 16) & 255;
        int t[4];
#pragma unroll
        for (int k = 0; k < 4; k++) t[k] = tap6(sm[k], sm[k + 1], sm[k + 2], sm[k + 3], sm[k + 4], sm[k + 5]);
        Mw[slot] = qM;
        Bw[slot][0] = (uint32_t)(t[0] & 0xffff) | ((uint32_t)t[1] << 16);
        Bw[slot][1] = (uint32_t)(t[2] & 0xffff) | ((uint32_t)t[3] << 16);
    };
    auto b1 = [&](int i, int k) -> int { return __builtin_amdgcn_sbfe((int)Bw[i][k >> 1], 16 * (k & 1), 16); };
#pragma unroll
    for (int i = 0; i < 5; i++) { issue(i); absorb(i); }
    issue(5);
    uint8_t *pG = D.pl[0], *pB = D.pl[1], *pH = D.pl[2], *pJ = D.pl[3];
#pragma unroll 1
    for (int r = 0; r < PT_H; r++) {
        absorb(5);
        if (r + 1 < PT_H) issue(r + 6);
        uint32_t vb = 0, vh = 0, vj = 0;
#pragma unroll
        for (int k = 0; k < 4; k++) {
            const int sh = 8 * k;
            const int Hv = tap6((Mw[0] >> sh) & 255, (Mw[1] >> sh) & 255, (Mw[2] >> sh) & 255, (Mw[3] >> sh) & 255,
                                (Mw[4] >> sh) & 255, (Mw[5] >> sh) & 255);
            const int J = tap6(b1(0, k), b1(1, k), b1(2, k), b1(3, k), b1(4, k), b1(5, k));
            vb |= (uint32_t)clip1_shr(b1(2, k) + 16, 5) << sh;
            vh |= (uint32_t)clip1_shr(Hv + 16, 5) << sh;
            vj |= (uint32_t)clip1_shr(J + 512, 10) << sh;
        }
        const ptrdiff_t o = (ptrdiff_t)(ya + r) * D.ps + x0;
        *(uint32_t *)(pG + o) = Mw[2];
        *(uint32_t *)(pB + o) = vb;
        *(uint32_t *)(pH + o) = vh;
        *(uint32_t *)(pJ + o) = vj;
#pragma unroll
        for (int i = 0; i < 5; i++) { Mw[i] = Mw[i + 1]; Bw[i][0] = Bw[i + 1][0]; Bw[i][1] = Bw[i + 1][1]; }
    }
}

DEV void ref_planes_chroma(const PlanesLaunch &a, const PlanesDesc &D, int i) {
    const int cwc = a.cw / 2, chc = a.ch / 2;
    const int pw = cwc + 2 * H264MI_CPADX, ph = chc + 2 * H264MI_CPADY, q = pw / 4, strips = (ph + PT_H - 1) / PT_H;
    const int pl = i / (q * strips);
    if (pl >= 2) return;
    i -= pl * q * strips;
    const int st = i / q, xx = (i - st * q) * 4, x = xx - H264MI_CPADX;
    static_assert(H264MI_CPADX % 4 == 0, "chroma quads are dword-aligned");
    const uint8_t *base = D.src[D.parity ? (*D.parity & 1) : 0][1 + pl];
#pragma unroll 1
    for (int r = 0; r < PT_H; r++) {
        const int yy = st * PT_H + r;
        if (yy >= ph) break;
        const int y = yy - H264MI_CPADY;
        *(uint32_t *)(D.plc[pl] + (ptrdiff_t)y * D.psc + x) = planes_row_bytes(base + (size_t)clip3(0, chc - 1, y) * cwc, x, cwc);
    }
}

static void ref_planes_grid(int cw, int ch, int &gx, int &gy, int &ystrips) {
    const int quads = (cw + 2 * H264MI_LPADX) / 4;
    gx = (quads + PT_Q - 1) / PT_Q;
    ystrips = (ch + 2 * H264MI_LPADY + PT_H - 1) / PT_H;
    const int cq = 2 * ((cw / 2 + 2 * H264MI_CPADX) / 4) * ((ch / 2 + 2 * H264MI_CPADY + PT_H - 1) / PT_H);
    gy = ystrips + (cq + gx * PT_Q - 1) / (gx * PT_Q);
}
__global__ __launch_bounds__(PT_Q) void dec_planes_kernel(PlanesLaunch a) {
    const PlanesDesc &D = a.pd[blockIdx.z];
    if (D.active && *D.active == 0) return;
    if ((int)blockIdx.y >= a.ystrips) {
        ref_planes_chroma(a, D, (((int)blockIdx.y - a.ystrips) * (int)gridDim.x + (int)blockIdx.x) * PT_Q + (int)threadIdx.x);
        return;
    }
    const int cw = a.cw, ch = a.ch;
    const int q = (int)blockIdx.x * PT_Q + (int)threadIdx.x;
    if (q * 4 >= cw + 2 * H264MI_LPADX) return;
    const int x0 = q * 4 - H264MI_LPADX, ya = (int)blockIdx.y * PT_H - H264MI_LPADY;
    const uint8_t *ref = D.src[D.parity ? (*D.parity & 1) : 0][0];
    uint32_t v[PT_H];
#pragma unroll
    for (int r = 0; r < PT_H; r++) v[r] = planes_row_bytes(ref + (size_t)clip3(0, ch - 1, ya + r) * cw, x0, cw);
#pragma unroll
    for (int r = 0; r < PT_H; r++) *(uint32_t *)(D.pl[0] + (ptrdiff_t)(ya + r) * D.ps + x0) = v[r];
}
static int launch_dec_planes(int S, int cw, int ch, const PlanesDesc *pd, hipStream_t st) {
    int gx, gy, ystrips;
    ref_planes_grid(cw, ch, gx, gy, ystrips);
    const PlanesLaunch pla{S, cw, ch, pd, ystrips};
    hipLaunchKernelGGL(dec_planes_kernel, dim3(gx, gy, S), dim3(PT_Q), 0, st, pla);
    return hipGetLastError() == hipSuccess ? 0 : -1;
}

static_assert(PACK_THREADS == PT_Q, "enc_post_kernel: one block size");
struct PostLaunch { PackLaunch pk; PlanesLaunch pl; int gx, gy; };
__global__ __launch_bounds__(PT_Q) void enc_post_kernel(PostLaunch a) {
    const int b = (int)blockIdx.x;
    if (b < a.pk.S) { enc_pack_block(a.pk, b); return; }
    const int r = b - a.pk.S, per = a.gx * a.gy, z = r / per, yx = r - z * per, y = yx / a.gx;
    ref_planes_block(a.pl, yx - y * a.gx, y, z, a.gx);
}
__global__ __launch_bounds__(PT_Q) void enc_post_slices_kernel(PostLaunch a) {
    const int b = (int)blockIdx.x;
    if (b < a.pk.S) { enc_pack_block_slices(a.pk, b); return; }
    const int r = b - a.pk.S, per = a.gx * a.gy, z = r / per, yx = r - z * per, y = yx / a.gx;
    ref_planes_block(a.pl, yx - y * a.gx, y, z, a.gx);
}
static int launch_enc_post(const PackLaunch &pk, int cw, int ch, const PlanesDesc *pd, hipStream_t st, bool slices) {
    int gx, gy, ystrips;
    ref_planes_grid(cw, ch, gx, gy, ystrips);
    const PostLaunch pl{pk, PlanesLaunch{pk.S, cw, ch, pd, ystrips}, gx, gy};
    if (slices) hipLaunchKernelGGL(enc_post_slices_kernel, dim3(pk.S + gx * gy * pk.S), dim3(PT_Q), 0, st, pl);
    else hipLaunchKernelGGL(enc_post_kernel, dim3(pk.S + gx * gy * pk.S), dim3(PT_Q), 0, st, pl);
    return hipGetLastError() == hipSuccess ? 0 : -1;
}

}
```

openh264-wasm_amd/csrc/runtime_enc.inc:

```
#include <cstdio>
#include <cstdlib>
#include <cstring>
#include <vector>

namespace h264mi {

#define HIPCHECK(x)                                                                                   \
    do {                                                                                              \
        hipError_t e_ = (x);                                                                          \
        if (e_ != hipSuccess) {                                                                       \
            fprintf(stderr, "h264mi: %s failed: %s (%s:%d)\n", #x, hipGetErrorString(e_), __FILE__, __LINE__); \
            return -1;                                                                                \
        }                                                                                             \
    } while (0)

struct HostBits {
    std::vector<uint8_t> b;
    uint64_t acc = 0;
    int n = 0;
    void put(uint32_t v, int k) {
        if (k <= 0) return;
        if (k < 32) v &= (1u << k) - 1u;
        acc = (acc << k) | v; n += k;
        while (n >= 8) { n -= 8; b.push_back((uint8_t)(acc >> n)); }
    }
    void ue(uint32_t v) { uint64_t k = (uint64_t)v + 1; int l = 0; while ((k >> l) > 1) l++; put(0, l); put((uint32_t)k, l + 1); }
    void se(int v) { ue(v > 0 ? (uint32_t)(2 * v - 1) : (uint32_t)(-2 * v)); }
    void trailing() { put(1, 1); if (n) put(0, 8 - n); }
};
static size_t nal_wrap(uint8_t *out, int ref_idc, int type, const std::vector<uint8_t> &rbsp) {
    size_t o = 0;
    out[o++] = 0; out[o++] = 0; out[o++] = 0; out[o++] = 1;
    out[o++] = (uint8_t)((ref_idc << 5) | type);
    int z = 0;
    for (uint8_t c : rbsp) {
        if (z >= 2 && c <= 3) { out[o++] = 3; z = 0; }
        out[o++] = c;
        z = c == 0 ? z + 1 : 0;
    }
    return o;
}
static int level_idc_for(int w, int h, int bitrate, int *cs3) {
    static const int32_t L[17][5] = {
        {10, 1485, 99, 396, 64},       {9, 1485, 99, 396, 128},       {11, 3000, 396, 900, 192},
        {12, 6000, 396, 2376, 384},    {13, 11880, 396, 2376, 768},   {20, 11880, 396, 2376, 2000},
        {21, 19800, 792, 4752, 4000},  {22, 20250, 1620, 8100, 4000}, {30, 40500, 1620, 8100, 10000},
        {31, 108000, 3600, 18000, 14000}, {32, 216000, 5120, 20480, 20000}, {40, 245760, 8192, 32768, 20000},
        {41, 245760, 8192, 32768, 50000}, {42, 522240, 8704, 34816, 50000}, {50, 589824, 22080, 110400, 135000},
        {51, 983040, 36864, 184320, 240000}, {52, 2073600, 36864, 184320, 240000}};
    const uint32_t mbw = (uint32_t)(w + 15) >> 4, mbh = (uint32_t)(h + 15) >> 4, mbs = mbw * mbh;
    const uint32_t sq = mbw * mbw > mbh * mbh ? mbw * mbw : mbh * mbh;
    const uint32_t mbps = (uint32_t)(60.0f * (float)mbs);
    int level = 51;
    *cs3 = 0;
    for (auto &l : L) {
        if ((uint32_t)l[1] < mbps || (uint32_t)l[2] < mbs || ((uint32_t)l[2] << 3) < sq || (uint32_t)l[3] < mbs) continue;
        if (bitrate && l[4] * 1200 < bitrate) continue;
        level = l[0];
        break;
    }
    if (level == 9) { *cs3 = 1; level = 11; }
    return level;
}
static size_t write_sps(int w, int h, int bitrate, uint8_t *out) {
    int mbw = (w + 15) / 16, mbh = (h + 15) / 16, cs3;
    const int level = level_idc_for(w, h, bitrate, &cs3);
    HostBits b;
    b.put(66, 8); b.put(0xC0 | (cs3 << 4), 8); b.put(level, 8);
    b.ue(0); b.ue(15 - 4); b.ue(2); b.ue(1); b.put(0, 1);
    b.ue(mbw - 1); b.ue(mbh - 1); b.put(1, 1); b.put(level >= 30, 1);
    int crop = (mbw * 16 != w) || (mbh * 16 != h);
    b.put(crop, 1);
    if (crop) { b.ue(0); b.ue((mbw * 16 - w) / 2); b.ue(0); b.ue((mbh * 16 - h) / 2); }
    b.put(1, 1);
    b.put(0, 8);
    b.put(1, 1); b.put(1, 1);
    b.ue(0); b.ue(0); b.ue(16); b.ue(16); b.ue(0); b.ue(1);
    b.trailing();
    return nal_wrap(out, 3, 7, b.b);
}
static size_t write_pps(uint8_t *out) {
    HostBits b;
    b.ue(0); b.ue(0); b.put(0, 1); b.put(0, 1); b.ue(0); b.ue(0); b.ue(0); b.put(0, 1); b.put(0, 2);
    b.se(0); b.se(0); b.se(0); b.put(1, 1); b.put(0, 1); b.put(0, 1);
    b.trailing();
    return nal_wrap(out, 3, 8, b.b);
}
static void rc_seq_init(RcState &r, int w, int h, int bitrate) {
    static const double BPP[4][4] = {{0.25, 0.5, 0.75, 1.0}, {0.1, 0.2, 0.3, 0.4}, {0.03, 0.05, 0.09, 0.13}, {0.01, 0.03, 0.06, 0.1}};
    static const int INITQP[4][5] = {{34, 28, 26, 24, 22}, {36, 30, 28, 26, 24}, {36, 32, 30, 28, 26}, {36, 34, 32, 30, 28}};
    static const int RANGE[5][2] = {{40, 28}, {37, 25}, {36, 24}, {35, 23}, {34, 22}};
    auto clip = [](int lo, int hi, int v) { return v < lo ? lo : (v > hi ? hi : v); };
    memset(&r, 0, sizeof(r));
    const int w16 = (w + 15) & ~15, h16 = (h + 15) & ~15;
    r.mbw = w16 >> 4;
    r.nmb = r.mbw * (h16 >> 4);
    const bool narrow = r.mbw < 31;
    const int g0 = narrow ? 1 : 2, g1 = narrow ? 2 : 4;
    r.skip_qp = narrow ? 24 : 31;
    r.mb_per_gom = r.mbw * ((10 * (g1 - g0)) / 100 + g0);
    r.gom_count = (r.mb_per_gom + r.nmb - 1) / r.mb_per_gom;
    r.tl_weight = 2000;
    r.gop_num = 8;
    const float fps = 60.0f;
    r.c_bpf = (int)((fps * 0.5f + (float)bitrate) / fps);
    r.c_max_bits_tl = (int)(((int64_t)r.c_bpf * 150 * r.tl_weight + 100000) / 200000);
    r.c_min_bits_tl = (int)(((int64_t)r.c_bpf * (100 - ((100 - 10) >> 1)) * r.tl_weight + 100000) / 200000);
    r.c_buffer_size_skip = (int)((50 * (int64_t)bitrate + 50) / 100);
    const double bpp = (double)bitrate / (double)((fps * (float)w16) * (float)h16);
    const int area = w16 * h16;
    const int cls = area < 28801 ? 0 : ((unsigned)area < 115201u ? 1 : ((unsigned)area < 460801u ? 2 : 3));
    int i = 0;
    while (i < 4 && !(BPP[cls][i] >= bpp)) i++;
    r.idr_hi = clip(12, 42, RANGE[i][0]);
    r.idr_lo = clip(12, 42, RANGE[i][1]);
    r.idr_table_qp = INITQP[cls][i];
    r.skip_en = 1;
}

static void wait_limit_from_env() {
    const char *e = getenv("H264MI_WAIT_LIMIT_MS");
    if (!e) return;
    const long ms = atol(e);
    if (ms <= 0) return;
    const uint64_t ticks = (uint64_t)ms * 100000u;
    (void)hipMemcpyToSymbol(HIP_SYMBOL(g_wait_limit_ticks), &ticks, sizeof(ticks));
}

struct EncCtx {
    int w, h, mbw, mbh, nmb, cw, ch, S, bitrate;
    hipStream_t stream;
    bool own_stream;

    size_t fbytes;
    uint8_t *d_src = nullptr;
    uint8_t *d_pool = nullptr;
    EncState *d_st = nullptr;
    EncDesc *d_desc[2] = {nullptr, nullptr};
    DbkDesc *d_dbk[2] = {nullptr, nullptr};
    PlanesDesc *d_pd[2] = {nullptr, nullptr};
    uint32_t *d_ticket = nullptr;
    uint32_t *d_done = nullptr;
    int gom_count = 0, begin_k = 1;
    int gom_rows = 1;
    int sgrp = 0;
    bool gom_exact = false;
    int slices = 1;
    bool quality = false;
    h264mi_quality *d_qual = nullptr;
    std::vector<EncDesc> h_desc[2];
    int parity = 0;
    std::vector<uint8_t> h_out;
    bool timing = false;
    uint64_t *d_prof = nullptr;
    uint64_t *d_tl = nullptr;
    int dlag = 0;
    int prio = 0;
    int prof_row = -1;
    int lean = -1;
    int xq = 1;
    int ncu = 256;
    std::vector<hipEvent_t> ev;
    int ev_used = 0;
    std::vector<h264mi_overlay> ov;
    const uint8_t *ov_sprites = nullptr;
    int ov_w = 0, ov_h = 0;
};

struct EncMbLaunch {
    const uint8_t *src_base;
    size_t src_stride;
};

static void enc_free(EncCtx *c) {
    if (!c) return;

    for (auto e : c->ev) (void)hipEventDestroy(e);
    (void)hipFree(c->d_pool);
    (void)hipFree(c->d_qual);
    (void)hipFree(c->d_prof);
    (void)hipFree(c->d_tl);
    if (c->own_stream) (void)hipStreamDestroy(c->stream);
    delete c;
}

static int enc_set_quality(EncCtx *c, bool on) {
    if (c->w < 16 || c->h < 16) return -1;
    if (on && !c->quality) {
        if (!c->d_qual && hipMalloc(&c->d_qual, sizeof(h264mi_quality) * (size_t)c->S) != hipSuccess) { c->d_qual = nullptr; return -1; }
        if (hipMemsetAsync(c->d_qual, 0, sizeof(h264mi_quality) * (size_t)c->S, c->stream) != hipSuccess) return -1;
    }
    c->quality = on;
    return 0;
}

static bool slices_valid(int mbh, int n) { return n >= 1 && n <= mbh && n <= H264MI_MAX_SLICES; }

static EncCtx *enc_create(int w, int h, int bitrate, int S, hipStream_t stream) {
    if (w <= 0 || h <= 0 || (w & 1) || (h & 1) || S <= 0 || S > H264MI_MAX_STREAMS || w > 16 * H264MI_ENC_MAX_MBW || h > 4096) return nullptr;
    wait_limit_from_env();
    EncCtx *c = new EncCtx();
    c->w = w; c->h = h; c->mbw = (w + 15) / 16; c->mbh = (h + 15) / 16; c->nmb = c->mbw * c->mbh;
    c->cw = c->mbw * 16; c->ch = c->mbh * 16; c->S = S; c->bitrate = bitrate;
    c->fbytes = (size_t)w * h + 2 * (size_t)(w / 2) * (h / 2);
    if (stream) { c->stream = stream; c->own_stream = false; }
    else { if (hipStreamCreateWithFlags(&c->stream, hipStreamNonBlocking) != hipSuccess) { delete c; return nullptr; } c->own_stream = true; }
    const size_t ysz = (size_t)c->cw * c->ch, csz = ysz / 4, pic = ysz + 2 * csz;
    const size_t rbsp_dw = (size_t)c->nmb * H264MI_MB_SLOT_DWORDS + 1024;
    const size_t nal_cap = rbsp_dw * 4 * 3 / 2 + 4096;
    auto al = [](size_t x) { return (x + 255) & ~(size_t)255; };
    size_t off_rec = 0, off_ref0 = off_rec + al(pic), off_ref1 = off_ref0 + al(pic);
    size_t off_info = off_ref1 + al(pic), off_coef = off_info + al(sizeof(MbInfo) * c->nmb);
    size_t off_gran = off_coef + al(sizeof(MbCoef) * c->nmb);
    size_t off_dgran = off_gran + al(8 * (size_t)H264MI_GRANULES_PER_MB * c->nmb);
    size_t off_bits = off_dgran + al(8 * (size_t)H264MI_DBK_GRANULES_PER_MB * c->nmb);
    size_t off_len = off_bits + al(4 * (size_t)H264MI_MB_SLOT_DWORDS * c->nmb);
    size_t off_rbsp = off_len + al(4 * (size_t)c->nmb);
    size_t off_nal = off_rbsp + al(4 * rbsp_dw);
    const size_t lps = (size_t)c->cw + 2 * H264MI_LPADX, lph = (size_t)c->ch + 2 * H264MI_LPADY;
    const size_t cps = (size_t)c->cw / 2 + 2 * H264MI_CPADX, cph = (size_t)c->ch / 2 + 2 * H264MI_CPADY;
    size_t off_pl = off_nal + al(nal_cap), off_plc = off_pl + 4 * al(lps * lph);
    size_t off_egr = off_plc + 2 * al(cps * cph);
    size_t off_rowqp = off_egr + al(8 * 128 * (size_t)c->nmb), off_rowbits = off_rowqp + al(4 * (size_t)c->mbh);
    size_t off_rowq = off_rowbits + al(4 * (size_t)c->mbh);
    if (const char *e = getenv("H264MI_GOM_EXACT")) c->gom_exact = atoi(e) != 0;
    if (const char *e = getenv("H264MI_ENC_SLICES")) {
        const int n = atoi(e);
        if (slices_valid(c->mbh, n) && !(c->gom_exact && n > 1)) c->slices = n;
    }
    RcState rc0;
    rc_seq_init(rc0, w, h, bitrate);
    c->gom_count = rc0.gom_count;
    c->begin_k = rc0.gom_count < 8 ? rc0.gom_count : 8;
    size_t off_psrc = off_rowq + al(8 * (size_t)c->mbh), off_gomc = off_psrc + 2 * al(ysz);
    size_t off_bitg = off_gomc + al(8 * (size_t)rc0.gom_count), off_gomst = off_bitg + al(8 * (size_t)c->nmb);
    size_t off_sks = off_gomst + al(32 * (size_t)rc0.gom_count);
    size_t per = off_sks + 2 * al(4 * ((size_t)c->nmb + 1));
    c->gom_rows = rc0.mb_per_gom / rc0.mbw;
    size_t hdr = al(sizeof(EncState) * S) + 2 * al(sizeof(EncDesc) * S) + 2 * al(sizeof(DbkDesc) * S) + 2 * al(sizeof(PlanesDesc) * S) + 256 + al(4 * (size_t)S);
    size_t total = hdr + al(c->fbytes * S) + per * S;
    if (hipMalloc(&c->d_pool, total) != hipSuccess) { if (c->own_stream) (void)hipStreamDestroy(c->stream); delete c; return nullptr; }
    (void)hipMemsetAsync(c->d_pool, 0, total, c->stream);
    uint8_t *p = c->d_pool;
    c->d_st = (EncState *)p; p += al(sizeof(EncState) * S);
    c->d_desc[0] = (EncDesc *)p; p += al(sizeof(EncDesc) * S);
    c->d_desc[1] = (EncDesc *)p; p += al(sizeof(EncDesc) * S);
    c->d_dbk[0] = (DbkDesc *)p; p += al(sizeof(DbkDesc) * S);
    c->d_dbk[1] = (DbkDesc *)p; p += al(sizeof(DbkDesc) * S);
    c->d_pd[0] = (PlanesDesc *)p; p += al(sizeof(PlanesDesc) * S);
    c->d_pd[1] = (PlanesDesc *)p; p += al(sizeof(PlanesDesc) * S);
    c->d_ticket = (uint32_t *)p; p += 256;
    c->d_done = (uint32_t *)p; p += al(4 * (size_t)S);
    c->d_src = p; p += al(c->fbytes * S);
    std::vector<EncState> hs(S);
    std::vector<DbkDesc> hd[2];
    std::vector<PlanesDesc> hp[2];
    uint8_t sps[64], pps[32];
    size_t nsps = write_sps(w, h, bitrate, sps), npps = write_pps(pps);
    for (int par = 0; par < 2; par++) { c->h_desc[par].resize(S); hd[par].resize(S); hp[par].resize(S); }
    for (int s = 0; s < S; s++) {
        uint8_t *b = p + per * s;
        uint8_t *rec = b + off_rec, *r0 = b + off_ref0, *r1 = b + off_ref1;
        for (int par = 0; par < 2; par++) {
            EncDesc &d = c->h_desc[par][s];
            uint8_t *ref = par == 0 ? r0 : r1, *dbk = par == 0 ? r1 : r0;
            d.src = nullptr;
            d.rec[0] = rec; d.rec[1] = rec + ysz; d.rec[2] = rec + ysz + csz;
            d.ref[0] = ref; d.ref[1] = ref + ysz; d.ref[2] = ref + ysz + csz;
            d.dbk[0] = dbk; d.dbk[1] = dbk + ysz; d.dbk[2] = dbk + ysz + csz;
            d.info = (MbInfo *)(b + off_info); d.coef = (MbCoef *)(b + off_coef);
            d.gran = (uint64_t *)(b + off_gran); d.dgran = (uint64_t *)(b + off_dgran);
            d.mbbits = (uint32_t *)(b + off_bits); d.mblen = (uint32_t *)(b + off_len);
            d.rbsp = (uint32_t *)(b + off_rbsp); d.nal = b + off_nal;
            d.st = c->d_st + s; d.nal_cap = (int)nal_cap; d.rbsp_cap = (int)rbsp_dw;
            for (int k = 0; k < 4; k++) d.pl[k] = b + off_pl + k * al(lps * lph) + H264MI_LPADY * lps + H264MI_LPADX;
            for (int k = 0; k < 2; k++) d.plc[k] = b + off_plc + k * al(cps * cph) + H264MI_CPADY * cps + H264MI_CPADX;
            d.ps = (int)lps; d.psc = (int)cps; d.pad3[0] = d.pad3[1] = 0;
            d.egran = (uint64_t *)(b + off_egr);
            d.rowqp = (int32_t *)(b + off_rowqp); d.rowbits = (int32_t *)(b + off_rowbits); d.rowq = (uint64_t *)(b + off_rowq);
            d.psrc[0] = b + off_psrc; d.psrc[1] = b + off_psrc + al(ysz);
            d.gomc = (uint32_t *)(b + off_gomc);
            d.bitg = (uint64_t *)(b + off_bitg); d.gomst = (uint64_t *)(b + off_gomst);
            int32_t *sk0 = (int32_t *)(b + off_sks), *sk1 = (int32_t *)(b + off_sks + al(4 * ((size_t)c->nmb + 1)));
            d.sksad_ref = par == 0 ? sk0 : sk1; d.sksad_cur = par == 0 ? sk1 : sk0;
            DbkDesc &k = hd[par][s];
            for (int i = 0; i < 3; i++) { k.rec[i] = d.rec[i]; k.out[0][i] = d.dbk[i]; k.out[1][i] = d.dbk[i]; }
            k.info = d.info; k.dgran = d.dgran; k.epoch = &c->d_st[s].epoch; k.disable = nullptr;
            k.active = nullptr; k.parity = nullptr; k.abort_word = &c->d_st[s].err; k.src_gran = d.egran;
            PlanesDesc &pd = hp[par][s];
            for (int i = 0; i < 3; i++) pd.src[0][i] = pd.src[1][i] = d.dbk[i];
            pd.parity = nullptr; pd.active = nullptr;
            for (int k2 = 0; k2 < 4; k2++) pd.pl[k2] = d.pl[k2];
            pd.plc[0] = d.plc[0]; pd.plc[1] = d.plc[1]; pd.ps = d.ps; pd.psc = d.psc;
        }
        EncState &st = hs[s];
        memset(&st, 0, sizeof(st));
        st.rc = rc0;
        st.first = 1; st.idr_pic_id = 0; st.bitrate = bitrate;
        st.cur_slices = c->slices;
        std::vector<int32_t> rq((size_t)c->mbh, 0);
        (void)hipMemcpyAsync(b + off_rowqp, rq.data(), 4 * (size_t)c->mbh, hipMemcpyHostToDevice, c->stream);
        (void)hipStreamSynchronize(c->stream);
        st.sps_bytes = (int)nsps; st.pps_bytes = (int)npps;
        memcpy(st.sps, sps, nsps); memcpy(st.pps, pps, npps);
    }
    (void)hipMemcpyAsync(c->d_st, hs.data(), sizeof(EncState) * S, hipMemcpyHostToDevice, c->stream);
    for (int par = 0; par < 2; par++) {
        (void)hipMemcpyAsync(c->d_desc[par], c->h_desc[par].data(), sizeof(EncDesc) * S, hipMemcpyHostToDevice, c->stream);
        (void)hipMemcpyAsync(c->d_dbk[par], hd[par].data(), sizeof(DbkDesc) * S, hipMemcpyHostToDevice, c->stream);
        (void)hipMemcpyAsync(c->d_pd[par], hp[par].data(), sizeof(PlanesDesc) * S, hipMemcpyHostToDevice, c->stream);
    }
    if (hipStreamSynchronize(c->stream) != hipSuccess) { enc_free(c); return nullptr; }
    if (const char *e = getenv("H264MI_DBK_LAG")) c->dlag = atoi(e);
    if (const char *e = getenv("H264MI_ENC_PRIO")) c->prio = atoi(e);
    if (const char *e = getenv("H264MI_ENC_PROF_ROW")) c->prof_row = atoi(e);
    if (const char *e = getenv("H264MI_ENC_LEAN")) c->lean = atoi(e);
    if (const char *e = getenv("H264MI_ENC_XQ")) c->xq = atoi(e);
    if (const char *e = getenv("H264MI_ENC_SGRP")) c->sgrp = atoi(e);
    {
        int dev = 0, n = 0;
        if (hipGetDevice(&dev) == hipSuccess && hipDeviceGetAttribute(&n, hipDeviceAttributeMultiprocessorCount, dev) == hipSuccess && n > 0)
            c->ncu = n;
    }
    if (const char *e = getenv("H264MI_ENC_QUALITY")) (void)enc_set_quality(c, atoi(e) != 0);
    if (getenv("H264MI_ENC_TL") && hipMalloc(&c->d_tl, 4 * (size_t)S * c->mbh * sizeof(uint64_t)) == hipSuccess)
        (void)hipMemset(c->d_tl, 0, 4 * (size_t)S * c->mbh * sizeof(uint64_t));
    if (getenv("H264MI_ENC_PROF") && hipMalloc(&c->d_prof, 64 * sizeof(uint64_t)) == hipSuccess)
        (void)hipMemset(c->d_prof, 0, 64 * sizeof(uint64_t));
    return c;
}

int launch_quality_enc(h264mi_quality *d_out, const uint8_t *d_frames, size_t fbytes, int w, int h, int cw, const EncDesc *desc, int S,
                       hipStream_t s);
int launch_quality_i420(h264mi_quality *d_out, const uint8_t *a, const uint8_t *b, int w, int h, int n, hipStream_t s);
bool quality_args_ok(int w, int h, int n);
int launch_scale_i420(uint8_t *dst, int dw, int dh, const uint8_t *src, int sw, int sh, int n, hipStream_t s);
bool scale_args_ok(int dw, int dh, int sw, int sh, int n);
bool scale_ranges_overlap(const void *dst, int dw, int dh, const void *src, int sw, int sh, int n);
int launch_compose_i420(uint8_t *dst, int cw, int ch, const uint8_t *src, int src_w, int src_h, const h264mi_cell *cells, int ncells,
                        hipStream_t s);
int launch_fill_i420(uint8_t *dst, int w, int h, int n, int y, int cb, int cr, hipStream_t s);
bool compose_args_ok(int cw, int ch, int ncanvas, int src_w, int src_h, int nsrc, const h264mi_cell *cells, int ncells);
bool compose_ranges_overlap(const void *canvas, int cw, int ch, int ncanvas, const void *src, int src_w, int src_h, int nsrc);
bool fill_args_ok(int w, int h, int n, int y, int cb, int cr);
int mosaic_cells(h264mi_cell *out, int cap, int n, int src_w, int src_h, int cw, int ch);
int launch_overlay_i420(uint8_t *dst, int cw, int ch, const uint8_t *spr, int ow, int oh, const h264mi_overlay *ov, int nov, hipStream_t s);
int launch_rgba_to_i420a(const uint8_t *d_rgba, int w, int h, int n, uint8_t *d_out, hipStream_t s);
bool overlay_args_ok(int cw, int ch, int ncanvas, int ow, int oh, int nsprites, const h264mi_overlay *ov, int nov);
bool overlay_ranges_overlap(const void *canvas, int cw, int ch, int ncanvas, const void *spr, int ow, int oh, int nsprites);
bool rgba_to_i420a_args_ok(int w, int h, int n);
int launch_upscale_i420(uint8_t *dst, int dw, int dh, const uint8_t *src, int sw, int sh, int n, int filter, hipStream_t s);
bool upscale_args_ok(int dw, int dh, int sw, int sh, int n, int filter);
bool upscale_ranges_overlap(const void *dst, int dw, int dh, const void *src, int sw, int sh, int n);
int launch_compose_any_i420(uint8_t *dst, int cw, int ch, const uint8_t *src, int src_w, int src_h, const h264mi_cell *cells, int ncells,
                            int filter, hipStream_t s);
bool compose_any_args_ok(int cw, int ch, int ncanvas, int src_w, int src_h, int nsrc, const h264mi_cell *cells, int ncells, int filter);
int speaker_cells(h264mi_cell *out, int cap, int n, int speaker, int src_w, int src_h, int cw, int ch);

static int enc_frame(EncCtx *c, const uint8_t *d_frames) {
    const int par = c->parity;
    const int src_vec = (c->w % 16) == 0 && (c->fbytes % 16) == 0 && ((uintptr_t)d_frames % 16) == 0;
    hipLaunchKernelGGL(enc_begin_kernel, dim3(c->begin_k, c->S), dim3(256), 0, c->stream,
                       BeginLaunch{c->S, c->w, c->h, c->cw, c->ch, c->begin_k, c->d_desc[par], c->d_ticket, d_frames, c->fbytes, src_vec, c->d_done, c->slices});
    EncLaunch el{c->w, c->h, c->mbw, c->mbh, c->S, c->d_desc[par], c->d_ticket, d_frames, c->fbytes, c->d_prof, src_vec,
                 c->d_dbk[par], c->d_prof ? c->d_prof + 16 : nullptr, c->dlag};
    if (c->timing) {
        if (c->ev_used + 2 > (int)c->ev.size()) {
            for (int i = 0; i < 64; i++) { hipEvent_t e; HIPCHECK(hipEventCreate(&e)); c->ev.push_back(e); }
        }
        HIPCHECK(hipEventRecord(c->ev[c->ev_used], c->stream));
    }
    const bool lean = c->lean >= 0 ? c->lean != 0 : c->S * c->mbh >= 2 * c->ncu;
    if (c->xq != 0 && c->S % 8 == 0 && (c->dlag <= 0 || c->gom_exact)) el.xq = 8;
    el.tl = c->d_tl;
    el.prio = c->prio;
    el.prof_row = c->prof_row;
    if (c->gom_exact) { el.gomr = c->gom_rows; el.dlag = 0; }
    el.sgrp = c->sgrp;
    if (lean) hipLaunchKernelGGL(enc_mb_kernel<true>, dim3(2 * c->S * c->mbh), dim3(ENC_THREADS), 0, c->stream, el);
    else hipLaunchKernelGGL(enc_mb_kernel<false>, dim3(2 * c->S * c->mbh), dim3(ENC_THREADS), 0, c->stream, el);
    if (c->timing) { HIPCHECK(hipEventRecord(c->ev[c->ev_used + 1], c->stream)); c->ev_used += 2; }
    if (launch_enc_post(PackLaunch{c->mbw, c->mbh, c->S, c->d_desc[par]}, c->cw, c->ch, c->d_pd[par], c->stream, c->slices > 1) != 0) return -1;
    HIPCHECK(hipGetLastError());
    if (c->quality && launch_quality_enc(c->d_qual, d_frames, c->fbytes, c->w, c->h, c->cw, c->d_desc[par], c->S, c->stream) != 0) return -1;
    c->parity ^= 1;
    return 0;
}

}

namespace h264mi {
struct PackNalLaunch { int S; const EncDesc *desc; uint8_t *dst; int slot; int32_t *sizes; };
__global__ __launch_bounds__(256) void enc_copy_nals_kernel(PackNalLaunch a) {
    const int s = blockIdx.y;
    if (s >= a.S) return;
    const EncDesc &D = a.desc[s];
    int n = D.st->nal_bytes;
    if (n > a.slot) { if (blockIdx.x == 0 && threadIdx.x == 0) D.st->err = 4; n = a.slot; }
    if (a.sizes && blockIdx.x == 0 && threadIdx.x == 0) a.sizes[s] = n;
    uint8_t *o = a.dst + (size_t)s * a.slot;
    for (int i = (blockIdx.x * blockDim.x + threadIdx.x) * 4; i < n; i += gridDim.x * blockDim.x * 4) {
        if (i + 4 <= n) *(uint32_t *)(o + i) = *(const uint32_t *)(D.nal + i);
        else for (int k = i; k < n; k++) o[k] = D.nal[k];
    }
}
}
```

Measured before the change: 5596.

## Compute half-pel planes on demand in LDS tiles instead of precomputed global planes

Stops precomputing the three half-pel interpolated reference planes (b, h, j) across the whole frame. Only the integer-pel plane is kept in global memory and the LDS window. When a fractional motion vector is evaluated, the workgroup builds an 18x18 tile of b/h/j samples around it in LDS. This cuts plane-kernel work, global memory traffic and LDS footprint, and shrinks EncLds so more workgroups fit per CU. The cost is extra interpolation math and barriers inside the motion-estimation loop. The ref_planes debug API now returns zeros for the removed planes.

```diff
diff --git a/openh264-wasm_amd/csrc/capi_enc.inc b/openh264-wasm_amd/csrc/capi_enc.inc
--- a/openh264-wasm_amd/csrc/capi_enc.inc
+++ b/openh264-wasm_amd/csrc/capi_enc.inc
@@ -309,8 +309,8 @@
     const size_t lsz = (size_t)d.ps * (e->c->ch + 2 * H264MI_LPADY), csz = (size_t)d.psc * (e->c->ch / 2 + 2 * H264MI_CPADY);
     uint8_t *o = (uint8_t *)host_out;
     if (hipStreamSynchronize(e->c->stream) != hipSuccess) return -1;
-    for (int k = 0; k < 4; k++)
-        if (hipMemcpy(o + k * lsz, d.pl[k] - (size_t)H264MI_LPADY * d.ps - H264MI_LPADX, lsz, hipMemcpyDeviceToHost) != hipSuccess) return -1;
+    if (hipMemcpy(o, d.pl[0] - (size_t)H264MI_LPADY * d.ps - H264MI_LPADX, lsz, hipMemcpyDeviceToHost) != hipSuccess) return -1;
+    memset(o + lsz, 0, 3 * lsz);
     for (int k = 0; k < 2; k++)
         if (hipMemcpy(o + 4 * lsz + k * csz, d.plc[k] - (size_t)H264MI_CPADY * d.psc - H264MI_CPADX, csz, hipMemcpyDeviceToHost) != hipSuccess) return -1;
     return 0;
diff --git a/openh264-wasm_amd/csrc/enc_mb.inc b/openh264-wasm_amd/csrc/enc_mb.inc
--- a/openh264-wasm_amd/csrc/enc_mb.inc
+++ b/openh264-wasm_amd/csrc/enc_mb.inc
@@ -9,9 +9,17 @@
 constexpr int WIN_STRIDE = WIN_RING + 4, WINC_STRIDE = WINC_RING + 4;
 DEV void win_put4(uint8_t *d, u32x4 v) { uint32_t *p = (uint32_t *)d; p[0] = v.x; p[1] = v.y; p[2] = v.z; p[3] = v.w; }
 DEV void win_put2(uint8_t *d, u32x2 v) { uint32_t *p = (uint32_t *)d; p[0] = v.x; p[1] = v.y; }
+constexpr int ME_RANGE = 16;
+constexpr int WIN_BACK = 24;
+constexpr int TILE_N = 18, TILE_STRIDE = 20, TB1_ROWS = TILE_N + 5;
+static_assert(-(ME_RANGE + 1) - 2 >= -WIN_BACK, "a tile build's first column / row is inside the window");
+static_assert(ME_RANGE + TILE_N + 2 < WIN_RING - WIN_BACK, "a tile build's last column / row is inside the window");
+static_assert(TILE_STRIDE % 4 == 0 && ((TILE_N - 4) >> 2) * 4 + 8 <= TILE_STRIDE, "tile4 reads two dwords inside a row");
 constexpr int ENC_CROSS_THR = 1024;
 struct EncLds {
-    alignas(16) uint8_t win[4][64 * WIN_STRIDE];
+    alignas(16) uint8_t win[64 * WIN_STRIDE];
+    alignas(4) uint8_t tile[3][TILE_N * TILE_STRIDE];
+    alignas(4) int16_t tb1[TB1_ROWS * TILE_N];
     alignas(16) uint8_t winc[2][32 * WINC_STRIDE];
     alignas(16) uint8_t src[256];
     alignas(16) uint8_t srcc[2][64];
@@ -88,11 +96,14 @@
 
 DEV int tap6(int a, int b, int c, int d, int e, int f) { return a - 5 * b + 20 * c + 20 * d - 5 * e + f; }
 
-DEV int Wpl(const EncLds &S, int p, int Y0, int gx, int gy) { return S.win[p][(gy - Y0) * WIN_STRIDE + ((gx + 24) & (WIN_RING - 1))]; }
+DEV int Wg(const EncLds &S, int Y0, int gx, int gy) { return S.win[(gy - Y0) * WIN_STRIDE + ((gx + WIN_BACK) & (WIN_RING - 1))]; }
+DEV int Wpl(const EncLds &S, int p, int Y0, int TX, int TY, int gx, int gy) {
+    return p == 0 ? Wg(S, Y0, gx, gy) : (int)S.tile[p - 1][(gy - TY) * TILE_STRIDE + (gx - TX)];
+}
 #define AVG(a, b) (((a) + (b) + 1) >> 1)
-DEV int Wsample(const EncLds &S, int Y0, int gx, int gy, int fx, int fy) {
+DEV int Wsample(const EncLds &S, int Y0, int TX, int TY, int gx, int gy, int fx, int fy) {
     const QSel q = qsel(fy * 4 + fx);
-    return AVG(Wpl(S, q.p1, Y0, gx + q.dx1, gy + q.dy1), Wpl(S, q.p2, Y0, gx + q.dx2, gy + q.dy2));
+    return AVG(Wpl(S, q.p1, Y0, TX, TY, gx + q.dx1, gy + q.dy1), Wpl(S, q.p2, Y0, TX, TY, gx + q.dx2, gy + q.dy2));
 }
 
 DEV int chroma_mc_sample(const EncLds &S, int mbx, int mvx, int mvy, int pl, int x, int y) {
diff --git a/openh264-wasm_amd/csrc/enc_mb_kernel.inc b/openh264-wasm_amd/csrc/enc_mb_kernel.inc
--- a/openh264-wasm_amd/csrc/enc_mb_kernel.inc
+++ b/openh264-wasm_amd/csrc/enc_mb_kernel.inc
@@ -357,21 +357,46 @@
     const int mx = n == 2 ? amx : (n == 3 ? bmx : cmx), my = n == 2 ? amy : (n == 3 ? bmy : cmy);
     const bool ok = n == 2 ? okA : (n == 3 ? okB : okC);
     const int vx = n == 0 ? p0 : (n == 1 ? 0 : mx), vy = n == 0 ? p1 : (n == 1 ? 0 : my);
-    cx = clip3(-16, 16, (vx + 2) >> 2); cy = clip3(-16, 16, (vy + 2) >> 2);
+    cx = clip3(-ME_RANGE, ME_RANGE, (vx + 2) >> 2); cy = clip3(-ME_RANGE, ME_RANGE, (vy + 2) >> 2);
     return n < 2 || ok;
 }
 DEV int mvbits(int mx, int my, const int mvp[2]) { return se_len(mx - mvp[0]) + se_len(my - mvp[1]); }
 
-DEV uint32_t win4(const EncLds &S, int p, int wr, int gx) {
-    const int sl = (gx + 24) & 63;
-    const uint32_t *row = (const uint32_t *)&S.win[p][wr * WIN_STRIDE];
-    return __builtin_amdgcn_alignbyte(row[((sl >> 2) + 1) & 15], row[sl >> 2], sl & 3);
+DEV uint32_t win4(const EncLds &S, int p, int Y0, int TX, int TY, int gy, int gx) {
+    if (p == 0) {
+        const int sl = (gx + WIN_BACK) & 63;
+        const uint32_t *row = (const uint32_t *)&S.win[(gy - Y0) * WIN_STRIDE];
+        return __builtin_amdgcn_alignbyte(row[((sl >> 2) + 1) & 15], row[sl >> 2], sl & 3);
+    }
+    const int tc = gx - TX;
+    const uint32_t *row = (const uint32_t *)&S.tile[p - 1][(gy - TY) * TILE_STRIDE];
+    return __builtin_amdgcn_alignbyte(row[(tc >> 2) + 1], row[tc >> 2], tc & 3);
+}
+DEV void tile_build(EncLds &S, int Y0, int TX, int TY) {
+    for (int i = e_tid(); i < TB1_ROWS * TILE_N; i += ENC_THREADS) {
+        const int r = i / TILE_N, gx = TX + (i - r * TILE_N), gy = TY - 2 + r;
+        S.tb1[i] = (int16_t)tap6(Wg(S, Y0, gx - 2, gy), Wg(S, Y0, gx - 1, gy), Wg(S, Y0, gx, gy), Wg(S, Y0, gx + 1, gy),
+                                 Wg(S, Y0, gx + 2, gy), Wg(S, Y0, gx + 3, gy));
+    }
+    lds_barrier();
+    for (int i = e_tid(); i < TILE_N * TILE_N; i += ENC_THREADS) {
+        const int r = i / TILE_N, c = i - r * TILE_N, gx = TX + c, gy = TY + r;
+        const int16_t *b1 = &S.tb1[i];
+        const int hv = tap6(Wg(S, Y0, gx, gy - 2), Wg(S, Y0, gx, gy - 1), Wg(S, Y0, gx, gy), Wg(S, Y0, gx, gy + 1),
+                            Wg(S, Y0, gx, gy + 2), Wg(S, Y0, gx, gy + 3));
+        const int jv = tap6(b1[0], b1[TILE_N], b1[2 * TILE_N], b1[3 * TILE_N], b1[4 * TILE_N], b1[5 * TILE_N]);
+        const int o = r * TILE_STRIDE + c;
+        S.tile[0][o] = (uint8_t)clip1_shr(b1[2 * TILE_N] + 16, 5);
+        S.tile[1][o] = (uint8_t)clip1_shr(hv + 16, 5);
+        S.tile[2][o] = (uint8_t)clip1_shr(jv + 512, 10);
+    }
+    lds_barrier();
 }
 DEV int sad16_row_group(const EncLds &S, int Y0, int X, int Y, int cx, int cy) {
     const int row = e_tid() & 15;
     const u32x4 sv = *(const u32x4 *)&S.src[row * 16];
-    const int sl = (X + cx + 24) & 63, i0 = sl >> 2, sh = sl & 3;
-    const uint32_t *rw = (const uint32_t *)&S.win[0][(Y + cy + row - Y0) * WIN_STRIDE];
+    const int sl = (X + cx + WIN_BACK) & 63, i0 = sl >> 2, sh = sl & 3;
+    const uint32_t *rw = (const uint32_t *)&S.win[(Y + cy + row - Y0) * WIN_STRIDE];
     const uint32_t w0 = rw[i0], w1 = rw[(i0 + 1) & 15], w2 = rw[(i0 + 2) & 15], w3 = rw[(i0 + 3) & 15], w4 = rw[(i0 + 4) & 15];
     uint32_t acc = __builtin_amdgcn_sad_u8(sv.x, __builtin_amdgcn_alignbyte(w1, w0, sh), 0u);
     acc = __builtin_amdgcn_sad_u8(sv.y, __builtin_amdgcn_alignbyte(w2, w1, sh), acc);
@@ -379,7 +404,7 @@
     acc = __builtin_amdgcn_sad_u8(sv.w, __builtin_amdgcn_alignbyte(w4, w3, sh), acc);
     return group16_sum((int)acc);
 }
-template <int N> DEV void satd16_mv_n(const EncLds &S, int Y0, int X, int Y, const int *mvx, const int *mvy, int *out) {
+template <int N> DEV void satd16_mv_n(const EncLds &S, int Y0, int TX, int TY, int X, int Y, const int *mvx, const int *mvy, int *out) {
     const int lane = e_tid() & 63, blk = lane >> 2, row = lane & 3;
     const int y = (blk >> 2) * 4 + row, x0 = (blk & 3) * 4;
     const uint32_t sv = *(const uint32_t *)&S.src[y * 16 + x0];
@@ -388,8 +413,8 @@
 #pragma unroll
     for (int n = 0; n < N; n++) {
         const QSel q = qsel((mvy[n] & 3) * 4 + (mvx[n] & 3));
-        const int gx = X + x0 + (mvx[n] >> 2), wr = Y + y + (mvy[n] >> 2) - Y0;
-        const uint32_t pa = win4(S, q.p1, wr + q.dy1, gx + q.dx1), pb = win4(S, q.p2, wr + q.dy2, gx + q.dx2);
+        const int gx = X + x0 + (mvx[n] >> 2), gy = Y + y + (mvy[n] >> 2);
+        const uint32_t pa = win4(S, q.p1, Y0, TX, TY, gy + q.dy1, gx + q.dx1), pb = win4(S, q.p2, Y0, TX, TY, gy + q.dy2, gx + q.dx2);
         const uint32_t pv = (pa | pb) - (((pa ^ pb) & 0xFEFEFEFEu) >> 1);
         const int d0 = (int)(sv & 255) - (int)(pv & 255), d1 = (int)((sv >> 8) & 255) - (int)((pv >> 8) & 255);
         const int d2 = (int)((sv >> 16) & 255) - (int)((pv >> 16) & 255), d3 = (int)(sv >> 24) - (int)(pv >> 24);
@@ -407,11 +432,6 @@
 #pragma unroll
     for (int n = 0; n < N; n++) out[n] = lane_read(acc[n], 0) + lane_read(acc[n], 16) + lane_read(acc[n], 32) + lane_read(acc[n], 48);
 }
-DEV int satd16_mv(const EncLds &S, int Y0, int X, int Y, int mvx, int mvy) {
-    int r;
-    satd16_mv_n<1>(S, Y0, X, Y, &mvx, &mvy, &r);
-    return r;
-}
 #define PSKIP_MV_MIN (-29)
 #define PSKIP_MV_MAX_LOW 12
 #define PSKIP_MAX_LEVEL 1
@@ -428,10 +448,10 @@
     const int t0 = 65535 / q.mf0 - q.fp0, t1 = (65535 / q.mf1 - q.fp1) >> 2, t2 = (65535 / q.mf2 - q.fp2) >> 1;
     return min(t0, min(t1, t2));
 }
-DEV void pskip_luma(EncLds &S, const Xf &X, const QuantQP &q, int Y0, int MX, int MY, int mvx, int mvy, int lb, int &lsad, int &ctr,
-                    bool &rej) {
+DEV void pskip_luma(EncLds &S, const Xf &X, const QuantQP &q, int Y0, int TX, int TY, int MX, int MY, int mvx, int mvy, int lb, int &lsad,
+                    int &ctr, bool &rej) {
     const int pos = e_lane() & 15, lx = (lb & 3) * 4 + (pos & 3), ly = (lb >> 2) * 4 + (pos >> 2);
-    const int pv = Wsample(S, Y0, MX + lx + (mvx >> 2), MY + ly + (mvy >> 2), mvx & 3, mvy & 3);
+    const int pv = Wsample(S, Y0, TX, TY, MX + lx + (mvx >> 2), MY + ly + (mvy >> 2), mvx & 3, mvy & 3);
     S.pred[ly * 16 + lx] = (uint8_t)pv;
     const int dl = S.src[ly * 16 + lx] - pv;
     const int bs = group16_sum(iabs(dl));
@@ -477,22 +497,22 @@
         if (r) atomicOr(&J[0], 1);
     }
 }
-DEV void pskip_judge_4w(EncLds &S, int *J, const Xf &X, int qp, int Y0, int MX, int MY, int mbx, int mvx, int mvy) {
+DEV void pskip_judge_4w(EncLds &S, int *J, const Xf &X, int qp, int Y0, int TX, int TY, int MX, int MY, int mbx, int mvx, int mvy) {
     const int w = e_wave(), g = e_lane() >> 4;
     const QuantQP q = make_qqp(qp), qc = make_qqp(c_CHROMA_QP[qp]);
     int lsad = 0, csad = 0, ctr = 0;
     bool rej = false;
-    pskip_luma(S, X, q, Y0, MX, MY, mvx, mvy, 4 * w + g, lsad, ctr, rej);
+    pskip_luma(S, X, q, Y0, TX, TY, MX, MY, mvx, mvy, 4 * w + g, lsad, ctr, rej);
     if (w < 2) pskip_chroma(S, X, qc, mbx, mvx, mvy, w, csad, rej);
     pskip_publish(J, lsad, csad, ctr, rej);
 }
-DEV void pskip_judge_3w(EncLds &S, int *J, const Xf &X, int qp, int Y0, int MX, int MY, int mbx, int mvx, int mvy) {
+DEV void pskip_judge_3w(EncLds &S, int *J, const Xf &X, int qp, int Y0, int TX, int TY, int MX, int MY, int mbx, int mvx, int mvy) {
     const int w = e_wave(), g = e_lane() >> 4;
     const QuantQP q = make_qqp(qp), qc = make_qqp(c_CHROMA_QP[qp]);
     int lsad = 0, csad = 0, ctr = 0;
     bool rej = false;
-    pskip_luma(S, X, q, Y0, MX, MY, mvx, mvy, 4 * (w - 1) + g, lsad, ctr, rej);
-    if (w == 1) pskip_luma(S, X, q, Y0, MX, MY, mvx, mvy, 12 + g, lsad, ctr, rej);
+    pskip_luma(S, X, q, Y0, TX, TY, MX, MY, mvx, mvy, 4 * (w - 1) + g, lsad, ctr, rej);
+    if (w == 1) pskip_luma(S, X, q, Y0, TX, TY, MX, MY, mvx, mvy, 12 + g, lsad, ctr, rej);
     else pskip_chroma(S, X, qc, mbx, mvx, mvy, w - 2, csad, rej);
     pskip_publish(J, lsad, csad, ctr, rej);
 }
@@ -506,9 +526,9 @@
     lds_barrier();
     return uni(J[1]);
 }
-DEV void fill_pred_mv(EncLds &S, int Y0, int X, int Y, int mvx, int mvy) {
+DEV void fill_pred_mv(EncLds &S, int Y0, int TX, int TY, int X, int Y, int mvx, int mvy) {
     const int i = e_tid();
-    S.pred[i] = (uint8_t)Wsample(S, Y0, X + (i & 15) + (mvx >> 2), Y + (i >> 4) + (mvy >> 2), mvx & 3, mvy & 3);
+    S.pred[i] = (uint8_t)Wsample(S, Y0, TX, TY, X + (i & 15) + (mvx >> 2), Y + (i >> 4) + (mvy >> 2), mvx & 3, mvy & 3);
 }
 
 #define CAND(k) uni(S.cand[k])
@@ -540,12 +560,19 @@
 #ifndef H264MI_ENC_WPE
 #define H264MI_ENC_WPE 4
 #endif
+#ifndef H264MI_ENC_GWAVE
+#define H264MI_ENC_GWAVE 3
+#endif
+#ifndef H264MI_ENC_CWAVE
+#define H264MI_ENC_CWAVE 3
+#endif
+static_assert(H264MI_ENC_CWAVE != 1, "wave 1's pfa holds the source rows");
 template <bool LEAN>
 __global__ __launch_bounds__(ENC_THREADS)
 __attribute__((amdgpu_waves_per_eu(LEAN && H264MI_ENC_WPE > 0 ? H264MI_ENC_WPE : 1, LEAN && H264MI_ENC_WPE > 0 ? H264MI_ENC_WPE : 8)))
 void enc_mb_kernel(EncLaunch a) {
     struct DbkCavlcLds { DbkLds d; CavlcTabs T; CavlcWaveLds w[2]; };
-    static_assert(sizeof(DbkCavlcLds) <= sizeof(EncLds), "the deblocking workgroup fits the encoder's LDS");
+    static_assert(sizeof(DbkCavlcLds) <= 16384 && sizeof(EncLds) <= 16384, "four workgroups per CU stay far inside the LDS");
     __shared__ union { EncLds e; DbkCavlcLds k; } SH;
     EncLds &S = SH.e;
     __shared__ int s_ticket;
@@ -695,14 +722,14 @@
     lds_barrier();
 
     const int ps = D.ps, psc = D.psc;
-    GLOBAL const uint8_t *plw = gbl(D.pl[tid >> 6]) + (ptrdiff_t)(Y0 + (tid & 63)) * ps;
+    GLOBAL const uint8_t *plw = gbl(D.pl[0]) + (ptrdiff_t)(Y0 + (tid & 63)) * ps;
     GLOBAL const uint8_t *plcw = gbl(D.plc[(tid >> 5) & 1]) + (ptrdiff_t)(mby * 8 - 12 + (tid & 31)) * psc;
     const bool vsrc = a.src_vec != 0;
     u32x4 pfw = {0, 0, 0, 0}, pfa = {0, 0, 0, 0};
     auto issue_prefetch = [&](int nx) {
         if (!idr) {
-            pfw = *(GLOBAL const u32x4 *)(plw + 16 * nx + 24);
-            if (wv == 0) pfa.xy = *(GLOBAL const u32x2 *)(plcw + 8 * nx + 12);
+            if (wv == H264MI_ENC_GWAVE) pfw = *(GLOBAL const u32x4 *)(plw + 16 * nx + 24);
+            if (wv == H264MI_ENC_CWAVE) pfa.xy = *(GLOBAL const u32x2 *)(plcw + 8 * nx + 12);
         }
         if (vsrc && wv == 1) {
             if (lane < 16) pfa = *(GLOBAL const u32x4 *)(srcY + (size_t)min(Y + lane, h - 1) * w + 16 * nx);
@@ -714,8 +741,8 @@
     };
     auto commit_prefetch = [&](int nx) {
         if (!idr) {
-            win_put4(&S.win[tid >> 6][(tid & 63) * WIN_STRIDE + ((16 * nx + 48) & 63)], pfw);
-            if (wv == 0) win_put2(&S.winc[lane >> 5][(lane & 31) * WINC_STRIDE + ((8 * nx + 24) & 31)], pfa.xy);
+            if (wv == H264MI_ENC_GWAVE) win_put4(&S.win[lane * WIN_STRIDE + ((16 * nx + 48) & 63)], pfw);
+            if (wv == H264MI_ENC_CWAVE) win_put2(&S.winc[lane >> 5][(lane & 31) * WINC_STRIDE + ((8 * nx + 24) & 31)], pfa.xy);
         }
         if (vsrc && wv == 1) {
             if (lane < 16) *(u32x4 *)&S.src[lane * 16] = pfa;
@@ -733,9 +760,7 @@
         }
     };
     if (!idr) {
-#pragma unroll
-        for (int k = 0; k < 4; k++)
-            win_put4(&S.win[tid >> 6][(tid & 63) * WIN_STRIDE + 16 * k], *(GLOBAL const u32x4 *)(plw - 24 + 16 * k));
+        win_put4(&S.win[(tid & 63) * WIN_STRIDE + 16 * (tid >> 6)], *(GLOBAL const u32x4 *)(plw - 24 + 16 * (tid >> 6)));
         if (wv == 0) {
 #pragma unroll
             for (int k = 0; k < 4; k++)
@@ -905,18 +930,32 @@
             const bool pred_skip = has_left ? L_skip : skB;
             const bool beside = try_skip && !pred_skip;
             bool skip_taken = false;
+            int tile_o = -1;
+#define TILE_X (X + (tile_o & 255) - 32)
+#define TILE_Y (Y + (tile_o >> 8) - 32)
+            auto tile_at = [&](int ox, int oy) {
+                const int o = uni((ox + 32) | ((oy + 32) << 8));
+                if (o != tile_o) { tile_o = o; tile_build(S, Y0, X + ox, Y + oy); }
+            };
+            auto tile_cover = [&](int mx, int my) {
+                if (((mx | my) & 3) == 0) return;
+                const int ix = mx >> 2, iy = my >> 2, dx = ix - ((tile_o & 255) - 32), dy = iy - ((tile_o >> 8) - 32);
+                if (tile_o < 0 || dx < 0 || dx > 1 || dy < 0 || dy > 1) tile_at(ix, iy);
+            };
             if (H264MI_ENC_LATE_PF == 2 && mbx + 1 < mbw) issue_prefetch(mbx + 1);
 #ifdef H264MI_ISA_MARK
             asm volatile(";;MARK_JUDGE" ::: "memory");
 #endif
             if (try_skip && pred_skip) {
-                pskip_judge_4w(S, J, XF, qp, Y0, X, Y, mbx, skmv[0], skmv[1]);
+                tile_cover(skmv[0], skmv[1]);
+                pskip_judge_4w(S, J, XF, qp, Y0, TILE_X, TILE_Y, X, Y, mbx, skmv[0], skmv[1]);
                 lds_barrier();
                 skip_taken = pskip_take();
             }
             const bool me_ran = !skip_taken;
             if (!skip_taken) {
                 if (!poll_above(false)) return;
+                if (beside) tile_cover(skmv[0], skmv[1]);
 #if H264MI_ENC_PH1 == 0
                 fill_top(false, false);
                 lds_barrier();
@@ -932,12 +971,12 @@
 #endif
                 if (wv != 0) {
 #if H264MI_ENC_PH1 == 0
-                    if (beside) pskip_judge_3w(S, J, XF, qp, Y0, X, Y, mbx, skmv[0], skmv[1]);
+                    if (beside) pskip_judge_3w(S, J, XF, qp, Y0, TILE_X, TILE_Y, X, Y, mbx, skmv[0], skmv[1]);
                     i16_sad_mode(S, k16, uni(wv - 1));
                     if (wv == (beside ? 3 : 1)) i16_sad_mode(S, k16, 3);
 #else
                     if (beside) {
-                        pskip_judge_3w(S, J, XF, qp, Y0, X, Y, mbx, skmv[0], skmv[1]);
+                        pskip_judge_3w(S, J, XF, qp, Y0, TILE_X, TILE_Y, X, Y, mbx, skmv[0], skmv[1]);
                         stamp(24 + wv, t_ph);
 #if H264MI_ENC_PH1 == 2
                         fill_top(true, false);
@@ -983,7 +1022,7 @@
                     for (int it = 0; it < 32; it++) {
                         const int cx = bx + (grp == 1 ? -1 : (grp == 2 ? 1 : 0)), cy = by + (grp == 0 ? -1 : (grp == 3 ? 1 : 0));
                         const int sad = sad16_row_group(S, Y0, X, Y, cx, cy);
-                        const bool ok = cx >= -16 && cx <= 16 && cy >= -16 && cy <= 16;
+                        const bool ok = cx >= -ME_RANGE && cx <= ME_RANGE && cy >= -ME_RANGE && cy <= ME_RANGE;
                         const int k = wave_min(ok ? ((sad + lam * mvbits(4 * cx, 4 * cy, mvp)) << 2) | grp : 0x7fffffff);
                         if (k == 0x7fffffff || (k >> 2) >= bc) break;
                         bc = k >> 2;
@@ -1033,6 +1072,7 @@
             } else if (!skip_taken) {
                 int bx = uni(S.cand[17]), by = uni(S.cand[18]), bcf = uni(S.cand[19]);
                 if (uni(S.cand[19]) > ENC_CROSS_THR) {
+                    static_assert(ME_RANGE == 16, "the cross search's candidate numbering");
                     const int bc = uni(S.cand[19]);
                     int kl = 0x7fffffff;
 #pragma unroll 1
@@ -1058,6 +1098,7 @@
                 do_intra = c16 < bcf;
               if (!do_intra) {
                 const int wv4 = uni(tid >> 6);
+                tile_at(bx - 1, by - 1);
                 {
                     int mx[3], my[3], cv[3];
 #pragma unroll
@@ -1066,10 +1107,10 @@
                         mx[n] = 4 * bx + (k < 0 ? 0 : 2 * sub_dx(k & 7)); my[n] = 4 * by + (k < 0 ? 0 : 2 * sub_dy(k & 7));
                     }
                     if (wv4 == 0) {
-                        satd16_mv_n<3>(S, Y0, X, Y, mx, my, cv);
+                        satd16_mv_n<3>(S, Y0, TILE_X, TILE_Y, X, Y, mx, my, cv);
                         if (lane == 0) { S.cand[0] = cv[0]; S.cand[4] = cv[1]; S.cand[8] = cv[2]; }
                     } else {
-                        satd16_mv_n<2>(S, Y0, X, Y, mx, my, cv);
+                        satd16_mv_n<2>(S, Y0, TILE_X, TILE_Y, X, Y, mx, my, cv);
                         if (lane == 0) { S.cand[wv4] = cv[0]; S.cand[wv4 + 4] = cv[1]; }
                     }
                 }
@@ -1087,7 +1128,7 @@
                     int mx[2], my[2], cv[2];
 #pragma unroll
                     for (int n = 0; n < 2; n++) { mx[n] = 4 * bx + bdx + sub_dx(wv4 + 4 * n); my[n] = 4 * by + bdy + sub_dy(wv4 + 4 * n); }
-                    satd16_mv_n<2>(S, Y0, X, Y, mx, my, cv);
+                    satd16_mv_n<2>(S, Y0, TILE_X, TILE_Y, X, Y, mx, my, cv);
                     if (lane == 0) { S.cand[9 + wv4] = cv[0]; S.cand[13 + wv4] = cv[1]; }
                 }
                 lds_barrier();
@@ -1107,7 +1148,8 @@
                     const bool at_skmv = mvx == skmv[0] && mvy == skmv[1];
                     if (!at_skmv) publish_decision(type, mvx, mvy, -1);
                     mvdx = mvx - mvp[0]; mvdy = mvy - mvp[1];
-                    fill_pred_mv(S, Y0, X, Y, mvx, mvy);
+                    tile_cover(mvx, mvy);
+                    fill_pred_mv(S, Y0, TILE_X, TILE_Y, X, Y, mvx, mvy);
                     chroma_mc(S, mbx, mby, mvx, mvy);
                     lapf(15);
                     cbp = code_residual_nodc(S, XF, qp, 0, 1, true);
@@ -1312,6 +1354,8 @@
     }
     if (prof && tid < 40) atomicAdd((unsigned long long *)&a.prof[tid < 16 ? tid : tid + 16], (unsigned long long)s_prof[tid]);
     tl_end();
+#undef TILE_X
+#undef TILE_Y
 #undef tid
 #undef lane
 #undef above
diff --git a/openh264-wasm_amd/csrc/enc_planes.inc b/openh264-wasm_amd/csrc/enc_planes.inc
--- a/openh264-wasm_amd/csrc/enc_planes.inc
+++ b/openh264-wasm_amd/csrc/enc_planes.inc
@@ -17,59 +17,15 @@
         return;
     }
     const int cw = a.cw, ch = a.ch;
-    const int pw = cw + 2 * H264MI_LPADX;
     const int q = bx * PT_Q + (int)threadIdx.x;
-    if (q * 4 >= pw) return;
-    const int x0 = q * 4 - H264MI_LPADX;
-    const int ya = by * PT_H - H264MI_LPADY;
+    if (q * 4 >= cw + 2 * H264MI_LPADX) return;
+    const int x0 = q * 4 - H264MI_LPADX, ya = by * PT_H - H264MI_LPADY;
     const uint8_t *ref = D.src[D.parity ? (*D.parity & 1) : 0][0];
-    uint32_t Mw[6], Bw[6][2], qL, qM, qR;
-    auto issue = [&](int i) {
-        const uint8_t *row = ref + (size_t)clip3(0, ch - 1, ya - 2 + i) * cw;
-        qL = planes_row_bytes(row, x0 - 4, cw);
-        qM = planes_row_bytes(row, x0, cw);
-        qR = planes_row_bytes(row, x0 + 4, cw);
-    };
-    auto absorb = [&](int slot) {
-        const uint32_t lo = __builtin_amdgcn_alignbyte(qM, qL, 2), hi = __builtin_amdgcn_alignbyte(qR, qM, 2);
-        int sm[9];
-        sm[0] = lo & 255; sm[1] = (lo >> 8) & 255; sm[2] = (lo >> 16) & 255; sm[3] = lo >> 24;
-        sm[4] = hi & 255; sm[5] = (hi >> 8) & 255; sm[6] = (hi >> 16) & 255; sm[7] = hi >> 24; sm[8] = (qR >> 16) & 255;
-        int t[4];
+    uint32_t v[PT_H];
 #pragma unroll
-        for (int k = 0; k < 4; k++) t[k] = tap6(sm[k], sm[k + 1], sm[k + 2], sm[k + 3], sm[k + 4], sm[k + 5]);
-        Mw[slot] = qM;
-        Bw[slot][0] = (uint32_t)(t[0] & 0xffff) | ((uint32_t)t[1] << 16);
-        Bw[slot][1] = (uint32_t)(t[2] & 0xffff) | ((uint32_t)t[3] << 16);
-    };
-    auto b1 = [&](int i, int k) -> int { return __builtin_amdgcn_sbfe((int)Bw[i][k >> 1], 16 * (k & 1), 16); };
+    for (int r = 0; r < PT_H; r++) v[r] = planes_row_bytes(ref + (size_t)clip3(0, ch - 1, ya + r) * cw, x0, cw);
 #pragma unroll
-    for (int i = 0; i < 5; i++) { issue(i); absorb(i); }
-    issue(5);
-    uint8_t *pG = D.pl[0], *pB = D.pl[1], *pH = D.pl[2], *pJ = D.pl[3];
-#pragma unroll 1
-    for (int r = 0; r < PT_H; r++) {
-        absorb(5);
-        if (r + 1 < PT_H) issue(r + 6);
-        uint32_t vb = 0, vh = 0, vj = 0;
-#pragma unroll
-        for (int k = 0; k < 4; k++) {
-            const int sh = 8 * k;
-            const int Hv = tap6((Mw[0] >> sh) & 255, (Mw[1] >> sh) & 255, (Mw[2] >> sh) & 255, (Mw[3] >> sh) & 255,
-                                (Mw[4] >> sh) & 255, (Mw[5] >> sh) & 255);
-            const int J = tap6(b1(0, k), b1(1, k), b1(2, k), b1(3, k), b1(4, k), b1(5, k));
-            vb |= (uint32_t)clip1_shr(b1(2, k) + 16, 5) << sh;
-            vh |= (uint32_t)clip1_shr(Hv + 16, 5) << sh;
-            vj |= (uint32_t)clip1_shr(J + 512, 10) << sh;
-        }
-        const ptrdiff_t o = (ptrdiff_t)(ya + r) * D.ps + x0;
-        *(uint32_t *)(pG + o) = Mw[2];
-        *(uint32_t *)(pB + o) = vb;
-        *(uint32_t *)(pH + o) = vh;
-        *(uint32_t *)(pJ + o) = vj;
-#pragma unroll
-        for (int i = 0; i < 5; i++) { Mw[i] = Mw[i + 1]; Bw[i][0] = Bw[i + 1][0]; Bw[i][1] = Bw[i + 1][1]; }
-    }
+    for (int r = 0; r < PT_H; r++) *(uint32_t *)(D.pl[0] + (ptrdiff_t)(ya + r) * D.ps + x0) = v[r];
 }
 
 DEV void ref_planes_chroma(const PlanesLaunch &a, const PlanesDesc &D, int i) {
@@ -98,22 +54,7 @@
     gy = ystrips + (cq + gx * PT_Q - 1) / (gx * PT_Q);
 }
 __global__ __launch_bounds__(PT_Q) void dec_planes_kernel(PlanesLaunch a) {
-    const PlanesDesc &D = a.pd[blockIdx.z];
-    if (D.active && *D.active == 0) return;
-    if ((int)blockIdx.y >= a.ystrips) {
-        ref_planes_chroma(a, D, (((int)blockIdx.y - a.ystrips) * (int)gridDim.x + (int)blockIdx.x) * PT_Q + (int)threadIdx.x);
-        return;
-    }
-    const int cw = a.cw, ch = a.ch;
-    const int q = (int)blockIdx.x * PT_Q + (int)threadIdx.x;
-    if (q * 4 >= cw + 2 * H264MI_LPADX) return;
-    const int x0 = q * 4 - H264MI_LPADX, ya = (int)blockIdx.y * PT_H - H264MI_LPADY;
-    const uint8_t *ref = D.src[D.parity ? (*D.parity & 1) : 0][0];
-    uint32_t v[PT_H];
-#pragma unroll
-    for (int r = 0; r < PT_H; r++) v[r] = planes_row_bytes(ref + (size_t)clip3(0, ch - 1, ya + r) * cw, x0, cw);
-#pragma unroll
-    for (int r = 0; r < PT_H; r++) *(uint32_t *)(D.pl[0] + (ptrdiff_t)(ya + r) * D.ps + x0) = v[r];
+    ref_planes_block(a, (int)blockIdx.x, (int)blockIdx.y, (int)blockIdx.z, (int)gridDim.x);
 }
 static int launch_dec_planes(int S, int cw, int ch, const PlanesDesc *pd, hipStream_t st) {
     int gx, gy, ystrips;
diff --git a/openh264-wasm_amd/csrc/runtime_enc.inc b/openh264-wasm_amd/csrc/runtime_enc.inc
--- a/openh264-wasm_amd/csrc/runtime_enc.inc
+++ b/openh264-wasm_amd/csrc/runtime_enc.inc
@@ -219,7 +219,7 @@
     size_t off_nal = off_rbsp + al(4 * rbsp_dw);
     const size_t lps = (size_t)c->cw + 2 * H264MI_LPADX, lph = (size_t)c->ch + 2 * H264MI_LPADY;
     const size_t cps = (size_t)c->cw / 2 + 2 * H264MI_CPADX, cph = (size_t)c->ch / 2 + 2 * H264MI_CPADY;
-    size_t off_pl = off_nal + al(nal_cap), off_plc = off_pl + 4 * al(lps * lph);
+    size_t off_pl = off_nal + al(nal_cap), off_plc = off_pl + al(lps * lph);
     size_t off_egr = off_plc + 2 * al(cps * cph);
     size_t off_rowqp = off_egr + al(8 * 128 * (size_t)c->nmb), off_rowbits = off_rowqp + al(4 * (size_t)c->mbh);
     size_t off_rowq = off_rowbits + al(4 * (size_t)c->mbh);
@@ -273,7 +273,8 @@
             d.mbbits = (uint32_t *)(b + off_bits); d.mblen = (uint32_t *)(b + off_len);
             d.rbsp = (uint32_t *)(b + off_rbsp); d.nal = b + off_nal;
             d.st = c->d_st + s; d.nal_cap = (int)nal_cap; d.rbsp_cap = (int)rbsp_dw;
-            for (int k = 0; k < 4; k++) d.pl[k] = b + off_pl + k * al(lps * lph) + H264MI_LPADY * lps + H264MI_LPADX;
+            d.pl[0] = b + off_pl + H264MI_LPADY * lps + H264MI_LPADX;
+            d.pl[1] = d.pl[2] = d.pl[3] = nullptr;
             for (int k = 0; k < 2; k++) d.plc[k] = b + off_plc + k * al(cps * cph) + H264MI_CPADY * cps + H264MI_CPADX;
             d.ps = (int)lps; d.psc = (int)cps; d.pad3[0] = d.pad3[1] = 0;
             d.egran = (uint64_t *)(b + off_egr);
```

Result: no change. 5607 (median of 6 runs) (+0.2%).
